# rageworx/libsrcnn

Measured on AMD Instinct MI355X. Metric: megapixels/sec SRCNN Y-channel (2x upscale), higher is better.
Workload: dtype f32

## Files before the change

### include/srcnn_amd_debug.h

```cpp
#ifndef SRCNN_AMD_DEBUG_H
#define SRCNN_AMD_DEBUG_H

#include "srcnn_amd.h"

#ifdef __cplusplus
extern "C" {
#endif
#pragma GCC visibility push(default)

#define SRCNN_MODE_RELAXED  3
#define SRCNN_RELAX_L1      1u
#define SRCNN_RELAX_L2      2u
#define SRCNN_RELAX_L3_X64  4u
#define SRCNN_RELAX_L3_F32  8u

int         srcnn_set_relaxation(unsigned mask);

int srcnn_axis_table(int filter, unsigned dst_len, unsigned src_len, int* left, int* right, double* weights);

int srcnn_fused_diag(const float* d_up, unsigned w, unsigned h, float* d_out, unsigned long long* d_dbg, void* stream);

int srcnn_debug_counts(int* tables, int* lanes);

int srcnn_debug_settings(char* buf, size_t cap, int markdown);

int srcnn_debug_clock_probe(int on);
int srcnn_debug_clock_read(int context, unsigned long long* cycles, unsigned long long* ticks, int cap);

int srcnn_debug_band_plan(unsigned r0, unsigned r1, unsigned dw, int one_of_many, unsigned* cuts, int cap);

int srcnn_debug_process_phases(double* ms, int cap);

int srcnn_debug_stream_mode(unsigned* graph_frames, unsigned* plain_frames, int* fell_back);

#pragma GCC visibility pop
#ifdef __cplusplus
}
#endif
#endif
```

### libsrcnn_amd/__init__.py

```python
import ctypes as C
import os

import numpy as np

_HERE = os.path.dirname(os.path.abspath(__file__))
LIB_PATH = os.environ.get("SRCNN_AMD_LIB") or os.path.join(_HERE, "lib", "libsrcnn_amd.so")

SRCNNF_Nearest, SRCNNF_Bilinear, SRCNNF_Bicubic, SRCNNF_Lanczos3, SRCNNF_Bspline = range(5)
MODE_STRICT, MODE_FAST, MODE_FAST_F16, MODE_RELAXED = 0, 1, 2, 3
RELAX_L1, RELAX_L2, RELAX_L3_X64, RELAX_L3_F32 = 1, 2, 4, 8

STABLE_ABI_SYMBOLS = [
    "srcnn_abi_version", "srcnn_device_count", "srcnn_init", "srcnn_init_devices", "srcnn_context_count",
    "srcnn_context_device", "srcnn_set_context", "srcnn_get_context", "srcnn_shutdown", "srcnn_trim",
    "srcnn_last_error", "srcnn_set_mode", "srcnn_get_mode", "srcnn_device_name", "srcnn_set_workspace_limit",
    "srcnn_dev_alloc", "srcnn_dev_free", "srcnn_host_alloc_pinned", "srcnn_host_free_pinned", "srcnn_memcpy_h2d",
    "srcnn_memcpy_d2h", "srcnn_memset_dev", "srcnn_stream_create", "srcnn_stream_destroy", "srcnn_stream_sync",
    "srcnn_device_sync", "srcnn_event_create", "srcnn_event_destroy", "srcnn_event_record",
    "srcnn_stream_wait_event", "srcnn_event_elapsed_ms", "srcnn_profile_enable", "srcnn_profile_reset",
    "srcnn_profile_read", "srcnn_profile_read_context", "srcnn_y_upscale2x_f32_dev",
    "srcnn_y_upscale2x_f32_batch_dev", "srcnn_y_upscale2x_f32_band_dev", "srcnn_y_upscale2x_f32_node_dev",
    "srcnn_batch_graph_create", "srcnn_batch_graph_launch", "srcnn_batch_graph_destroy", "srcnn_y_path_f32_dev",
    "srcnn_resample_f32_dev", "srcnn_conv1_f32_dev", "srcnn_conv2_f32_dev", "srcnn_conv3_f32_dev",
    "srcnn_conv12_f32_dev", "srcnn_y_upscale2x_f32", "srcnn_y_upscale2x_f32_batch", "srcnn_y_upscale2x_f32_stream",
    "srcnn_y_path_f32", "srcnn_process_u8", "srcnn_process_u8_begin", "srcnn_process_u8_wait", "srcnn_delete_array",
    "srcnn_output_size", "srcnn_comm_unique_id", "srcnn_comm_init", "srcnn_comm_destroy", "srcnn_comm_rank",
    "srcnn_comm_gather_f32", "srcnn_comm_gatherv_f32", "srcnn_comm_gatherv_at_f32",
    "srcnn_comm_tiled_y_upscale2x_f32_dev", "srcnn_band_rows", "srcnn_tiled_piece", "srcnn_comm_allgather_f32",
    "srcnn_comm_barrier", "srcnn_comm_wait", "srcnn_comm_set_timeout_ms",
]
DEBUG_SYMBOLS = [
    "srcnn_set_relaxation", "srcnn_axis_table", "srcnn_fused_diag", "srcnn_debug_counts", "srcnn_debug_settings",
    "srcnn_debug_clock_probe", "srcnn_debug_clock_read", "srcnn_debug_band_plan", "srcnn_debug_process_phases", "srcnn_debug_stream_mode",
]
YUV_SYMBOLS = ["srcnn_yuv_abi_version", "srcnn_yuv420_upscale_dev"]
YUV_EX_SYMBOLS = ["srcnn_yuv_ex_abi_version", "srcnn_yuv_plane_size", "srcnn_yuv_upscale_dev"]
RGB_SYMBOLS = ["srcnn_rgb_abi_version", "srcnn_rgb_plane_size", "srcnn_rgb_upscale_dev"]
C_ABI_SYMBOLS = STABLE_ABI_SYMBOLS + DEBUG_SYMBOLS + YUV_SYMBOLS + YUV_EX_SYMBOLS + RGB_SYMBOLS
CXX_SYMBOLS = ["_Z20ConfigureFilterSRCNN15SRCNNFilterTypeb", "_Z12ProcessSRCNNPKhjjjfRPhRjPS1_Pj"]


class YuvFormat(C.Structure):
    _fields_ = [("struct_size", C.c_uint), ("layout", C.c_int), ("chroma", C.c_int), ("depth", C.c_int), ("msb_aligned", C.c_int)]


class RgbFormat(C.Structure):
    _fields_ = [("struct_size", C.c_uint), ("layout", C.c_int), ("order", C.c_int), ("alpha", C.c_int), ("depth", C.c_int)]


class SrcnnError(RuntimeError):
    def __init__(self, code, msg):
        super().__init__("libsrcnn_amd error %d: %s" % (code, msg))
        self.code = code


_lib = None


def lib():
    global _lib
    if _lib is None:
        if not os.path.exists(LIB_PATH):
            raise ImportError("%s is missing -- run `python -m libsrcnn_amd.build` (hipcc, gfx950). "
                              "There is no CPU fallback." % LIB_PATH)
        L = C.CDLL(LIB_PATH)
        vp, u, f, sz, i = C.c_void_p, C.c_uint, C.c_float, C.c_size_t, C.c_int
        sig = {
            "srcnn_abi_version": (i, []), "srcnn_device_count": (i, []), "srcnn_init": (i, [i]),
            "srcnn_init_devices": (i, [C.POINTER(i), i]), "srcnn_context_count": (i, []), "srcnn_context_device": (i, [i]),
            "srcnn_set_context": (i, [i]), "srcnn_get_context": (i, []), "srcnn_trim": (i, []),
            "srcnn_y_upscale2x_f32_node_dev": (i, [vp, u, u, vp, i]),
            "srcnn_comm_gatherv_at_f32": (i, [vp, C.POINTER(sz), C.POINTER(sz), vp, i, vp]),
            "srcnn_comm_tiled_y_upscale2x_f32_dev": (i, [vp, u, u, vp, vp, i, i, vp]),
            "srcnn_band_rows": (i, [u, i, i, C.POINTER(u), C.POINTER(u)]),
            "srcnn_tiled_piece": (i, [u, u, i, i, i, i, C.POINTER(u), C.POINTER(u)]),
            "srcnn_debug_band_plan": (i, [u, u, u, i, C.POINTER(u), i]),
            "srcnn_shutdown": (None, []), "srcnn_last_error": (C.c_char_p, []), "srcnn_set_mode": (i, [i]),
            "srcnn_get_mode": (i, []), "srcnn_set_relaxation": (i, [u]), "srcnn_device_name": (i, [C.c_char_p, sz]),
            "srcnn_set_workspace_limit": (sz, [sz]),
            "srcnn_dev_alloc": (vp, [sz]), "srcnn_dev_free": (None, [vp]),
            "srcnn_host_alloc_pinned": (vp, [sz]), "srcnn_host_free_pinned": (None, [vp]),
            "srcnn_memcpy_h2d": (i, [vp, vp, sz, vp]), "srcnn_memcpy_d2h": (i, [vp, vp, sz, vp]),
            "srcnn_memset_dev": (i, [vp, i, sz, vp]),
            "srcnn_stream_create": (i, [C.POINTER(vp)]), "srcnn_stream_destroy": (i, [vp]),
            "srcnn_stream_sync": (i, [vp]), "srcnn_device_sync": (i, []),
            "srcnn_event_create": (i, [C.POINTER(vp)]), "srcnn_event_destroy": (i, [vp]),
            "srcnn_event_record": (i, [vp, vp]), "srcnn_event_elapsed_ms": (i, [vp, vp, C.POINTER(f)]),
            "srcnn_stream_wait_event": (i, [vp, vp]),
            "srcnn_profile_enable": (i, [i]), "srcnn_profile_reset": (i, []),
            "srcnn_profile_read": (i, [i, C.POINTER(C.c_double), C.POINTER(C.c_ulonglong)]),
            "srcnn_profile_read_context": (i, [i, i, C.POINTER(C.c_double), C.POINTER(C.c_ulonglong)]),
            "srcnn_y_upscale2x_f32_dev": (i, [vp, u, u, vp, vp]),
            "srcnn_y_upscale2x_f32_batch_dev": (i, [vp, u, u, u, vp, vp]),
            "srcnn_y_upscale2x_f32_band_dev": (i, [vp, u, u, u, u, vp, vp]),
            "srcnn_batch_graph_create": (i, [vp, u, u, u, vp, vp, C.POINTER(vp)]),
            "srcnn_batch_graph_launch": (i, [vp]), "srcnn_batch_graph_destroy": (i, [vp]),
            "srcnn_y_path_f32_dev": (i, [vp, u, u, u, u, i, vp, vp]),
            "srcnn_resample_f32_dev": (i, [vp, u, u, u, u, i, vp, vp]),
            "srcnn_conv1_f32_dev": (i, [vp, u, u, vp, vp]), "srcnn_conv2_f32_dev": (i, [vp, u, u, vp, vp]),
            "srcnn_conv3_f32_dev": (i, [vp, u, u, vp, vp]), "srcnn_conv12_f32_dev": (i, [vp, u, u, vp, vp]),
            "srcnn_y_upscale2x_f32": (i, [vp, u, u, vp]), "srcnn_y_upscale2x_f32_batch": (i, [vp, u, u, u, vp]),
            "srcnn_y_path_f32": (i, [vp, u, u, u, u, i, vp]),
            "srcnn_y_upscale2x_f32_stream": (i, [vp, u, u, u, vp, i]),
            "srcnn_process_u8": (i, [vp, u, u, u, f, i, vp, vp]),
            "srcnn_process_u8_begin": (i, [vp, u, u, u, f, i, vp, vp, C.POINTER(vp)]), "srcnn_process_u8_wait": (i, [vp]),
            "srcnn_delete_array": (None, [vp]),
            "srcnn_output_size": (i, [u, u, f, i, C.POINTER(u), C.POINTER(u)]),
            "srcnn_axis_table": (i, [i, u, u, vp, vp, vp]),
            "srcnn_comm_unique_id": (i, [vp]), "srcnn_comm_init": (i, [vp, i, i]), "srcnn_comm_destroy": (i, []),
            "srcnn_comm_gather_f32": (i, [vp, sz, vp, i, vp]), "srcnn_comm_allgather_f32": (i, [vp, sz, vp, vp]),
            "srcnn_comm_gatherv_f32": (i, [vp, C.POINTER(sz), vp, i, vp]),
            "srcnn_comm_rank": (i, [C.POINTER(i), C.POINTER(i)]),
            "srcnn_debug_counts": (i, [C.POINTER(i), C.POINTER(i)]),
            "srcnn_fused_diag": (i, [vp, u, u, vp, vp, vp]),
            "srcnn_debug_clock_probe": (i, [i]), "srcnn_debug_clock_read": (i, [i, vp, vp, i]),
            "srcnn_debug_settings": (i, [C.c_char_p, sz, i]),
            "srcnn_debug_process_phases": (i, [C.POINTER(C.c_double), i]),
            "srcnn_debug_stream_mode": (i, [C.POINTER(u), C.POINTER(u), C.POINTER(i)]),
            "srcnn_comm_barrier": (i, [vp]), "srcnn_comm_wait": (i, [vp]), "srcnn_comm_set_timeout_ms": (i, [i]),
            "srcnn_yuv_abi_version": (i, []),
            "srcnn_yuv420_upscale_dev": (i, [i, u, u, f, i, C.POINTER(vp), C.POINTER(sz), C.POINTER(vp), C.POINTER(sz), vp]),
            "srcnn_yuv_ex_abi_version": (i, []),
            "srcnn_yuv_plane_size": (i, [C.POINTER(YuvFormat), u, u, i, C.POINTER(u), C.POINTER(u), C.POINTER(sz)]),
            "srcnn_yuv_upscale_dev": (i, [C.POINTER(YuvFormat), u, u, f, i, C.POINTER(vp), C.POINTER(sz), C.POINTER(vp), C.POINTER(sz), vp]),
            "srcnn_rgb_abi_version": (i, []),
            "srcnn_rgb_plane_size": (i, [C.POINTER(RgbFormat), u, u, i, C.POINTER(u), C.POINTER(u), C.POINTER(sz)]),
            "srcnn_rgb_upscale_dev": (i, [C.POINTER(RgbFormat), u, u, f, i, C.POINTER(vp), C.POINTER(sz), C.POINTER(vp), C.POINTER(sz), vp, sz, vp]),
        }
        for name, (res, args) in sig.items():
            if name in DEBUG_SYMBOLS + YUV_SYMBOLS + YUV_EX_SYMBOLS + RGB_SYMBOLS and not hasattr(L, name) and os.environ.get("SRCNN_AMD_LIB"):
                continue
            fn = getattr(L, name)
            fn.restype, fn.argtypes = res, args
        cfg = getattr(L, CXX_SYMBOLS[0])
        cfg.restype, cfg.argtypes = None, [i, C.c_bool]
        prc = getattr(L, CXX_SYMBOLS[1])
        prc.restype = i
        prc.argtypes = [vp, u, u, u, f, C.POINTER(vp), C.POINTER(u), C.POINTER(vp), C.POINTER(u)]
        _lib = L
    return _lib


def check(rc):
    if rc != 0:
        raise SrcnnError(rc, lib().srcnn_last_error().decode("utf-8", "replace"))


def init(device=0):
    check(lib().srcnn_init(int(device)))


def init_devices(devices=None):
    if devices is None:
        check(lib().srcnn_init_devices(None, 0))
    else:
        arr = (C.c_int * len(devices))(*devices)
        check(lib().srcnn_init_devices(arr, len(devices)))
    return lib().srcnn_context_count()


def context_count():
    return lib().srcnn_context_count()


def set_context(k):
    prev = lib().srcnn_set_context(int(k))
    if prev < 0:
        raise SrcnnError(prev, lib().srcnn_last_error().decode())
    return prev


def shutdown():
    lib().srcnn_shutdown()


def device_count():
    return lib().srcnn_device_count()


def device_name():
    buf = C.create_string_buffer(256)
    check(lib().srcnn_device_name(buf, 256))
    return buf.value.decode()


def set_mode(mode):
    prev = lib().srcnn_set_mode(int(mode))
    if prev < 0:
        raise SrcnnError(prev, lib().srcnn_last_error().decode())
    return prev


def set_relaxation(mask):
    prev = lib().srcnn_set_relaxation(int(mask))
    if prev < 0:
        raise SrcnnError(prev, lib().srcnn_last_error().decode())
    return prev


def sync():
    check(lib().srcnn_device_sync())


STAGES = ("resample", "conv12", "conv3")


def profile_enable(on=True):
    return lib().srcnn_profile_enable(1 if on else 0)


def profile_reset():
    check(lib().srcnn_profile_reset())


def clock_probe(on=True):
    return lib().srcnn_debug_clock_probe(1 if on else 0)


def clock_read(context=0, cap=8192):
    cyc = np.zeros(cap, np.uint64); tk = np.zeros(cap, np.uint64)
    n = lib().srcnn_debug_clock_read(int(context), cyc.ctypes.data, tk.ctypes.data, cap)
    if n < 0:
        raise SrcnnError(n, lib().srcnn_last_error().decode())
    n = min(n, cap)
    t = np.maximum(tk[:n].astype(np.float64), 1.0)
    return [(float(c) / float(x) * 100.0, float(x) / 100.0) for c, x in zip(cyc[:n].astype(np.float64), t)]


def profile_read_context(k):
    out = {}
    for st, name in enumerate(STAGES):
        ms, n = C.c_double(), C.c_ulonglong()
        check(lib().srcnn_profile_read_context(int(k), st, C.byref(ms), C.byref(n)))
        out[name] = (ms.value, n.value)
    return out


def profile_read():
    out = {}
    for k, name in enumerate(STAGES):
        ms, n = C.c_double(0), C.c_ulonglong(0)
        check(lib().srcnn_profile_read(k, C.byref(ms), C.byref(n)))
        out[name] = (ms.value, n.value)
    return out


class DeviceBuffer:
    def __init__(self, nbytes):
        self.nbytes = int(nbytes)
        self.ptr = lib().srcnn_dev_alloc(self.nbytes)
        if not self.ptr:
            raise SrcnnError(-202, lib().srcnn_last_error().decode())

    @classmethod
    def from_numpy(cls, arr):
        arr = np.ascontiguousarray(arr)
        b = cls(arr.nbytes)
        check(lib().srcnn_memcpy_h2d(b.ptr, arr.ctypes.data, arr.nbytes, None))
        return b

    def upload(self, arr, offset=0):
        arr = np.ascontiguousarray(arr)
        assert offset + arr.nbytes <= self.nbytes
        check(lib().srcnn_memcpy_h2d(self.ptr + offset, arr.ctypes.data, arr.nbytes, None))

    def to_numpy(self, dtype, shape, offset=0):
        out = np.empty(shape, dtype)
        assert offset + out.nbytes <= self.nbytes
        check(lib().srcnn_memcpy_d2h(out.ctypes.data, self.ptr + offset, out.nbytes, None))
        return out

    def free(self):
        if self.ptr:
            lib().srcnn_dev_free(self.ptr)
            self.ptr = None

    def __del__(self):
        try:
            self.free()
        except Exception:
            pass


class Stream:
    def __init__(self):
        h = C.c_void_p()
        check(lib().srcnn_stream_create(C.byref(h)))
        self.handle = h.value

    def sync(self):
        check(lib().srcnn_stream_sync(self.handle))

    def destroy(self):
        if self.handle:
            check(lib().srcnn_stream_destroy(self.handle))
            self.handle = None


class Event:
    def __init__(self):
        h = C.c_void_p()
        check(lib().srcnn_event_create(C.byref(h)))
        self.handle = h.value

    def record(self, stream=None):
        check(lib().srcnn_event_record(self.handle, stream.handle if stream else None))

    def elapsed_ms(self, stop):
        ms = C.c_float()
        check(lib().srcnn_event_elapsed_ms(self.handle, stop.handle, C.byref(ms)))
        return ms.value


def _plane(a):
    a = np.ascontiguousarray(a, np.float32)
    assert a.ndim == 2, a.shape
    return a


def y_upscale2x(y):
    y = _plane(y)
    h, w = y.shape
    out = np.empty((2 * h, 2 * w), np.float32)
    check(lib().srcnn_y_upscale2x_f32(y.ctypes.data, w, h, out.ctypes.data))
    return out


def y_upscale2x_batch(frames):
    frames = np.ascontiguousarray(frames, np.float32)
    n, h, w = frames.shape
    out = np.empty((n, 2 * h, 2 * w), np.float32)
    check(lib().srcnn_y_upscale2x_f32_batch(frames.ctypes.data, w, h, n, out.ctypes.data))
    return out


def y_upscale2x_stream(frames, use_graph=True):
    frames = np.ascontiguousarray(frames, np.float32)
    n, h, w = frames.shape
    out = np.empty((n, 2 * h, 2 * w), np.float32)
    g = 1 if use_graph == "auto" else (int(use_graph) if isinstance(use_graph, int) and not isinstance(use_graph, bool) else (2 if use_graph else 0))
    check(lib().srcnn_y_upscale2x_f32_stream(frames.ctypes.data, w, h, n, out.ctypes.data, g))
    return out


def stream_mode():
    g, p, f = C.c_uint(0), C.c_uint(0), C.c_int(0)
    check(lib().srcnn_debug_stream_mode(C.byref(g), C.byref(p), C.byref(f)))
    return g.value, p.value, bool(f.value)


def y_path(y, dw, dh, filt=SRCNNF_Bicubic):
    y = _plane(y)
    h, w = y.shape
    out = np.empty((dh, dw), np.float32)
    check(lib().srcnn_y_path_f32(y.ctypes.data, w, h, dw, dh, filt, out.ctypes.data))
    return out


def y_upscale2x_band(y, row0, rows):
    y = _plane(y)
    h, w = y.shape
    din = DeviceBuffer.from_numpy(y)
    dout = DeviceBuffer(rows * 2 * w * 4)
    check(lib().srcnn_y_upscale2x_f32_band_dev(din.ptr, w, h, row0, rows, dout.ptr, None))
    sync()
    return dout.to_numpy(np.float32, (rows, 2 * w))


def _stage(fn, src, out_shape, *dims):
    src = np.ascontiguousarray(src, np.float32)
    din = DeviceBuffer.from_numpy(src)
    dout = DeviceBuffer(int(np.prod(out_shape)) * 4)
    check(fn(din.ptr, *dims, dout.ptr, None))
    sync()
    return dout.to_numpy(np.float32, out_shape)


def resample(y, dw, dh, filt=SRCNNF_Bicubic):
    y = _plane(y)
    h, w = y.shape
    src = DeviceBuffer.from_numpy(y)
    dst = DeviceBuffer(dw * dh * 4)
    check(lib().srcnn_resample_f32_dev(src.ptr, w, h, dw, dh, filt, dst.ptr, None))
    sync()
    return dst.to_numpy(np.float32, (dh, dw))


def conv1(y):
    y = _plane(y)
    h, w = y.shape
    return _stage(lib().srcnn_conv1_f32_dev, y, (64, h, w), w, h)


def conv2(c1):
    _, h, w = c1.shape
    return _stage(lib().srcnn_conv2_f32_dev, c1, (32, h, w), w, h)


def conv3(c2):
    _, h, w = c2.shape
    return _stage(lib().srcnn_conv3_f32_dev, c2, (h, w), w, h)


def conv12(y):
    y = _plane(y)
    h, w = y.shape
    return _stage(lib().srcnn_conv12_f32_dev, y, (32, h, w), w, h)


def axis_table(dst_len, src_len, filt=SRCNNF_Bicubic):
    win = lib().srcnn_axis_table(filt, dst_len, src_len, None, None, None)
    if win < 0:
        raise SrcnnError(win, lib().srcnn_last_error().decode())
    left = np.zeros(dst_len, np.int32)
    right = np.zeros(dst_len, np.int32)
    w = np.zeros((dst_len, win + 1), np.float64)
    lib().srcnn_axis_table(filt, dst_len, src_len, left.ctypes.data, right.ctypes.data, w.ctypes.data)
    return left, right, w


def output_size(w, h, multiply, stepscale=False):
    ow, oh = C.c_uint(0), C.c_uint(0)
    rc = lib().srcnn_output_size(w, h, float(np.float32(multiply)), 1 if stepscale else 0, C.byref(ow), C.byref(oh))
    if rc != 0:
        raise SrcnnError(rc, "srcnn_output_size")
    return ow.value, oh.value


def process_u8(rgb, multiply=2.0, filt=SRCNNF_Bicubic, want_conv=True):
    rgb = np.ascontiguousarray(rgb, np.uint8)
    h, w, d = rgb.shape
    m = np.float32(multiply)
    dw, dh = int(np.float32(w) * m), int(np.float32(h) * m)
    out = np.empty((dh, dw, d), np.uint8)
    conv = np.empty((dh, dw), np.uint8) if want_conv else None
    check(lib().srcnn_process_u8(rgb.ctypes.data, w, h, d, float(m), filt, out.ctypes.data,
                                 conv.ctypes.data if want_conv else None))
    return out, conv


YUV_I420, YUV_NV12 = 0, 1
_YUV_FORMATS = {"i420": YUV_I420, "nv12": YUV_NV12, YUV_I420: YUV_I420, YUV_NV12: YUV_NV12}


def yuv420_sizes(w, h, multiply):
    dw, dh = output_size(w, h, multiply)
    return (dw, dh), ((w + 1) // 2, (h + 1) // 2), ((dw + 1) // 2, (dh + 1) // 2)


def _addr(p):
    if p is None:
        return None
    if isinstance(p, tuple):
        base, off = p
        return _addr(base) + int(off)
    return p.ptr if isinstance(p, DeviceBuffer) else int(p)


def yuv420_upscale_dev(fmt, w, h, multiply, filt, src, src_pitch, dst, dst_pitch, stream=None):
    vp, sz = C.c_void_p, C.c_size_t
    s = (vp * 3)(*[_addr(p) for p in src])
    d = (vp * 3)(*[_addr(p) for p in dst])
    sp = (sz * 3)(*src_pitch) if src_pitch is not None else None
    dp = (sz * 3)(*dst_pitch) if dst_pitch is not None else None
    handle = stream.handle if isinstance(stream, Stream) else stream
    check(lib().srcnn_yuv420_upscale_dev(int(_YUV_FORMATS.get(fmt, fmt)), int(w), int(h), float(np.float32(multiply)), int(filt), s, sp,
                                         d, dp, handle))


def yuv420_upscale(y, u, v=None, multiply=2.0, filt=SRCNNF_Bicubic, fmt="i420", stream=None):
    fmt = _YUV_FORMATS[fmt.lower() if isinstance(fmt, str) else fmt]
    y = np.ascontiguousarray(y, np.uint8)
    h, w = y.shape
    (dw, dh), (cw, ch), (dcw, dch) = yuv420_sizes(w, h, multiply)
    if fmt == YUV_NV12:
        planes = [y, np.ascontiguousarray(u, np.uint8).reshape(ch, 2 * cw)]
        shapes = [(dh, dw), (dch, 2 * dcw)]
    else:
        planes = [y, np.ascontiguousarray(u, np.uint8), np.ascontiguousarray(v, np.uint8)]
        assert planes[1].shape == planes[2].shape == (ch, cw), (planes[1].shape, planes[2].shape, (ch, cw))
        shapes = [(dh, dw), (dch, dcw), (dch, dcw)]
    din = [DeviceBuffer.from_numpy(p) for p in planes]
    dout = [DeviceBuffer(int(np.prod(s))) for s in shapes]
    pad = [None] * (3 - len(planes))
    yuv420_upscale_dev(fmt, w, h, multiply, filt, din + pad, None, dout + pad, None, stream)
    if isinstance(stream, Stream):
        stream.sync()
    else:
        check(lib().srcnn_stream_sync(stream))
    return tuple(b.to_numpy(np.uint8, s) for b, s in zip(dout, shapes))


YUV_PLANAR, YUV_SEMIPLANAR = 0, 1
YUV_420, YUV_422, YUV_444 = 0, 1, 2
_YUV_LAYOUTS = {"planar": YUV_PLANAR, "semiplanar": YUV_SEMIPLANAR, YUV_PLANAR: YUV_PLANAR, YUV_SEMIPLANAR: YUV_SEMIPLANAR}
_YUV_CHROMAS = {"420": YUV_420, "422": YUV_422, "444": YUV_444, 420: YUV_420, 422: YUV_422, 444: YUV_444,
                YUV_420: YUV_420, YUV_422: YUV_422, YUV_444: YUV_444}


def yuv_format(layout="planar", chroma="420", depth=8, msb_aligned=False):
    layout = layout.lower() if isinstance(layout, str) else layout
    return YuvFormat(C.sizeof(YuvFormat), int(_YUV_LAYOUTS.get(layout, layout)), int(_YUV_CHROMAS.get(chroma, chroma)), int(depth),
                     int(msb_aligned))


def yuv_plane_size(fmt, w, h, plane):
    c, r, b = C.c_uint(0), C.c_uint(0), C.c_size_t(0)
    check(lib().srcnn_yuv_plane_size(C.byref(fmt), int(w), int(h), int(plane), C.byref(c), C.byref(r), C.byref(b)))
    return c.value, r.value, b.value


def yuv_plane_sizes(fmt, w, h, multiply):
    dw, dh = output_size(w, h, multiply)
    n = 2 if fmt.layout == YUV_SEMIPLANAR else 3
    return ((dw, dh), [yuv_plane_size(fmt, w, h, k) for k in range(n)], [yuv_plane_size(fmt, dw, dh, k) for k in range(n)])


def yuv_upscale_dev(fmt, w, h, multiply, filt, src, src_pitch, dst, dst_pitch, stream=None):
    vp, sz = C.c_void_p, C.c_size_t
    s = (vp * 3)(*[_addr(p) for p in src]) if src is not None else None
    d = (vp * 3)(*[_addr(p) for p in dst]) if dst is not None else None
    sp = (sz * 3)(*src_pitch) if src_pitch is not None else None
    dp = (sz * 3)(*dst_pitch) if dst_pitch is not None else None
    handle = stream.handle if isinstance(stream, Stream) else stream
    check(lib().srcnn_yuv_upscale_dev(C.byref(fmt) if fmt is not None else None, int(w), int(h), float(np.float32(multiply)),
                                      int(filt), s, sp, d, dp, handle))


def yuv_upscale(planes, layout="planar", chroma="420", depth=8, msb_aligned=False, multiply=2.0, filt=SRCNNF_Bicubic, stream=None):
    fmt = yuv_format(layout, chroma, depth, msb_aligned)
    dt = np.uint8 if depth == 8 else np.uint16
    y = np.ascontiguousarray(planes[0], dt)
    h, w = y.shape
    _, src_sizes, dst_sizes = yuv_plane_sizes(fmt, w, h, multiply)
    bps = np.dtype(dt).itemsize
    ins = [y] + [np.ascontiguousarray(p, dt).reshape(r, rb // bps) for p, (_c, r, rb) in zip(planes[1:], src_sizes[1:])]
    assert len(ins) == len(src_sizes), "%d planes given, the format has %d" % (len(ins), len(src_sizes))
    shapes = [(r, rb // bps) for (_c, r, rb) in dst_sizes]
    din = [DeviceBuffer.from_numpy(p) for p in ins]
    dout = [DeviceBuffer(max(1, int(np.prod(s)) * bps)) for s in shapes]
    pad = [None] * (3 - len(ins))
    yuv_upscale_dev(fmt, w, h, multiply, filt, din + pad, None, dout + pad, None, stream)
    if isinstance(stream, Stream):
        stream.sync()
    else:
        check(lib().srcnn_stream_sync(stream))
    return tuple(b.to_numpy(dt, s) for b, s in zip(dout, shapes))


RGB_INTERLEAVED, RGB_PLANAR = 0, 1
RGB_ORDER_RGB, RGB_ORDER_BGR = 0, 1
_RGB_LAYOUTS = {"interleaved": RGB_INTERLEAVED, "hwc": RGB_INTERLEAVED, "planar": RGB_PLANAR, "chw": RGB_PLANAR}
_RGB_ORDERS = {"rgb": RGB_ORDER_RGB, "rgba": RGB_ORDER_RGB, "bgr": RGB_ORDER_BGR, "bgra": RGB_ORDER_BGR}


def rgb_format(layout="interleaved", order="rgb", alpha=False, depth=8):
    layout = layout.lower() if isinstance(layout, str) else layout
    order = order.lower() if isinstance(order, str) else order
    return RgbFormat(C.sizeof(RgbFormat), int(_RGB_LAYOUTS.get(layout, layout)), int(_RGB_ORDERS.get(order, order)), int(alpha), int(depth))

# ... 208 lines not shown
```

### libsrcnn_amd/csrc/srcnn_capi.cpp

```cpp
#include <dlfcn.h>
#include <hip/hip_runtime.h>
#include <sys/prctl.h>
#include <sys/syscall.h>
#include <unistd.h>

#include <algorithm>
#include <cstdio>
#include <cstdlib>
#include <cstring>
#include <string>
#include <thread>

#include "resample_table.hpp"
#include <chrono>
#include <sys/auxv.h>
#include <unistd.h>

#include "srcnn_host.hpp"
#include "srcnn_yuv.h"
#include "srcnn_rgb.h"
#include "../../include/srcnn_amd_yuv.h"
#include "../../include/srcnn_amd_yuv_ex.h"
#include "../../include/srcnn_amd_rgb.h"

// ... 593 lines not shown
    if (spin_waits()) return hipEventSynchronize(e);
    const hipError_t r = poll_until_ready([&] {
        if (!query_guard) return hipEventQuery(e);
        std::lock_guard<std::mutex> lk(*query_guard);
        return hipEventQuery(e);
    });
    (void)hipGetLastError();
    return r;
}

hipError_t wait_stream(hipStream_t s)
{
    if (spin_waits()) return hipStreamSynchronize(s);
    const hipError_t r = poll_until_ready([&] { return hipStreamQuery(s); });
    (void)hipGetLastError();
    return r;
}

void parallel_memcpy(void* dst, const void* src, size_t n)
{
    const size_t kChunk = 4u << 20;
    unsigned nt = (unsigned)std::min<size_t>(8, n / kChunk);
    if (nt <= 1) { memcpy(dst, src, n); return; }
    std::vector<std::thread> th;
    const size_t per = ((n / nt) + 4095) & ~size_t(4095);
    size_t done = 0;
    try {
        for (unsigned t = 1; t < nt; ++t) {
            const size_t off = (size_t)t * per;
            if (off >= n) break;
            const size_t len = std::min(per, n - off);
            th.emplace_back([=] { memcpy((char*)dst + off, (const char*)src + off, len); });
            done = off + len;
        }
    } catch (...) {
        done = th.empty() ? 0 : done;
    }
    memcpy(dst, src, std::min(per, n));
    const size_t covered = th.empty() ? std::min(per, n) : done;
    if (covered < n) memcpy((char*)dst + covered, (const char*)src + covered, n - covered);
    for (auto& t : th) t.join();
}

void ProcLane::release_buffers()
{
    ws.release();
    if (pin_in) (void)hipHostFree(pin_in);
    if (pin_out) (void)hipHostFree(pin_out);
    pin_in = pin_out = nullptr; pin_in_n = pin_out_n = 0;
}

void ProcLane::release()
{
    release_buffers();
    for (auto e : band_events) (void)hipEventDestroy(e);
    band_events.clear();
    if (st) (void)hipStreamDestroy(st);
    if (copy_st) (void)hipStreamDestroy(copy_st);
    if (in_st) (void)hipStreamDestroy(in_st);
    st = copy_st = in_st = nullptr;
}

void NodeLane::release()
{
    ws.release();
    (void)hipFree(in); (void)hipFree(band);
    in = band = nullptr; in_n = band_n = 0;
    for (auto e : events) (void)hipEventDestroy(e);
    events.clear();
    if (st) (void)hipStreamDestroy(st);
    if (copy_st) (void)hipStreamDestroy(copy_st);
    st = copy_st = nullptr;
}

LaneLease::LaneLease(Ctx& c) : cx(&c)
{
    std::unique_lock<std::mutex> lk(c.lane_mu);
    for (;;) {
        for (auto& l : c.lanes)
            if (!l->busy) { lane = l.get(); break; }
        if (lane) break;
        if (c.lanes.size() < G.max_lanes) {
            auto l = std::make_unique<ProcLane>();
            if (hipStreamCreateWithFlags(&l->st, hipStreamNonBlocking) != hipSuccess ||
                hipStreamCreateWithFlags(&l->copy_st, hipStreamNonBlocking) != hipSuccess ||
                hipStreamCreateWithFlags(&l->in_st, hipStreamNonBlocking) != hipSuccess) {
                l->release();
                rc = fail(SRCNN_E_HIP, "could not create the streams of a ProcessSRCNN lane");
                return;
            }
            c.lanes.push_back(std::move(l));
            lane = c.lanes.back().get();
            break;
        }
        c.lane_cv.wait(lk);
    }
    lane->busy = true;
}

LaneLease::~LaneLease()
{
    if (!lane) return;
    (void)hipSetDevice(cx->device);
    (void)hipStreamSynchronize(lane->st);
    (void)hipStreamSynchronize(lane->copy_st);
    (void)hipStreamSynchronize(lane->in_st);
    { std::lock_guard<std::mutex> lk(cx->lane_mu); lane->busy = false; }
    cx->lane_cv.notify_one();
}

namespace {

struct StageTimer {
    Ctx& cx; hipStream_t s; int stage; hipEvent_t a = nullptr, b = nullptr; bool on;
    hipEvent_t take()
    {
        if (!cx.event_pool.empty()) { hipEvent_t e = cx.event_pool.back(); cx.event_pool.pop_back(); return e; }
        hipEvent_t e = nullptr;
        if (hipEventCreate(&e) != hipSuccess) return nullptr;
        return e;
    }
    StageTimer(int stage_, const Call& c) : cx(*c.cx), s(c.s), stage(stage_), on(c.timing && G.profiling.load(std::memory_order_relaxed))
    {
        if (!on) return;
        std::lock_guard<std::mutex> lk(cx.mu);
        a = take(); b = take();
        if (!a || !b) { on = false; return; }
        (void)hipEventRecord(a, s);
    }
    ~StageTimer()
    {
        if (!on) return;
        (void)hipEventRecord(b, s);
        std::lock_guard<std::mutex> lk(cx.mu);
        cx.spans.push_back(StageSpan{a, b, stage});
    }
};

void drain_spans_locked(Ctx& cx)
{
    for (auto& sp : cx.spans) {
        float ms = 0.f;
        if (hipEventSynchronize(sp.b) == hipSuccess && hipEventElapsedTime(&ms, sp.a, sp.b) == hipSuccess) {
            cx.stage_ms[sp.stage] += ms;
            cx.stage_n[sp.stage] += 1;
        }
        cx.event_pool.push_back(sp.a);
        cx.event_pool.push_back(sp.b);
    }
    cx.spans.clear();
}

void run_conv12(const Call& c, const float* Y, int W, int H, int y_row_base, int y_rows, float* C2, size_t plane, int row0,
                int rows)
{
    unsigned long long* clk = nullptr;
    if (G.clock_probe.load(std::memory_order_relaxed) && c.cx->clock_buf)
        clk = c.cx->clock_buf + 2 * (size_t)(c.cx->clock_n.fetch_add(1) % kClockSlots);
    unsigned* queue = nullptr;
    hipStreamCaptureStatus cap = hipStreamCaptureStatusNone;
    const bool foreign_capture = c.s && c.ws && !c.ws->frozen && hipStreamIsCapturing(c.s, &cap) == hipSuccess && cap == hipStreamCaptureStatusActive;
    if (foreign_capture) clk = nullptr;
    if (c.ws && settings().conv12_queue && !foreign_capture) {
        if (c.ws->queue && c.ws->queue_dirty) {
            if (hipMemsetAsync(c.ws->queue, 0, 2 * sizeof(unsigned), c.s) == hipSuccess) c.ws->queue_dirty = false;
            else (void)hipGetLastError();
        }
        if (!c.ws->queue && !c.ws->frozen) {
            void* q = nullptr;
            if (hipMalloc(&q, 2 * sizeof(unsigned)) == hipSuccess && hipMemsetAsync(q, 0, 2 * sizeof(unsigned), c.s) == hipSuccess) c.ws->queue = static_cast<unsigned*>(q);
            else { (void)hipFree(q); (void)hipGetLastError(); }
        }
        queue = c.ws->queue;
    }
    launch_conv12_mfma(Y, W, H, y_row_base, y_rows, C2, plane, row0, rows, c.relax(), c.cx->num_cus, c.s, clk, queue);
}

DevAxisTable view_of(const TableRef& t) { return t->view(); }

int resample_src_rows(Call& c, const YSource& src, unsigned sw, unsigned sh, unsigned dw, unsigned dh, int filter,
                      unsigned r0, unsigned r1, float* d_dst)
{
    Workspace& ws = *c.ws;
    hipStream_t s = c.s;
    const float* d_in = src.plane;
    if (sw == dw && sh == dh) {
        if (!d_in) return fail(SRCNN_E_UNSUPPORTED, "identity-size resample needs a float plane");
        HIP_TRY(hipMemcpyAsync(d_dst, d_in + (size_t)r0 * sw, sizeof(float) * (size_t)(r1 - r0) * sw,
                               hipMemcpyDeviceToDevice, s));
        return SRCNN_OK;
    }
    TableRef tv, th;
    int rc;
    if (dw > sw && sh != dh) {
        if ((rc = get_table(c, filter, dw, sw, th))) return rc;
        if ((rc = get_table(c, filter, dh, sh, tv))) return rc;
        if (!settings().resample_2pass &&
            launch_rs2d(src, sw, sh, d_dst, dw, dh, r0, r1 - r0, view_of(tv), view_of(th), s)) return SRCNN_OK;
    }
    if (!d_in) return fail(SRCNN_E_UNSUPPORTED, "this resample shape needs a float source plane");
    if (dw <= sw) {
        const float* mid = d_in;
        int mid_row_base = 0;
        if (sw != dw) {
            if ((rc = get_table(c, filter, dw, sw, th))) return rc;
            if (sh != dh) {
                if ((rc = get_table(c, filter, dh, sh, tv))) return rc;
                unsigned lo = 0, hi = sh;
                tv->source_span(r0, r1, lo, hi);
                hi = std::min(hi, sh);
                if (hi <= lo) return fail(SRCNN_E_UNSUPPORTED, "empty source span for rows [%u,%u)", r0, r1);
                if ((rc = grow_ws(ws, ws.tmp, ws.tmp_n, (size_t)dw * (hi - lo)))) return rc;
                launch_resample_rows(d_in + (size_t)lo * sw, sw, ws.tmp, dw, hi - lo, view_of(th), s);
                mid = ws.tmp;
                mid_row_base = (int)lo;
            } else {
                launch_resample_rows(d_in + (size_t)r0 * sw, sw, d_dst, dw, r1 - r0, view_of(th), s);
                return SRCNN_OK;
            }
        }
        if (!tv && (rc = get_table(c, filter, dh, sh, tv))) return rc;
        launch_resample_cols(mid, dw, mid_row_base, d_dst, r0, r1 - r0, view_of(tv), s);
    } else {
        if (!th && (rc = get_table(c, filter, dw, sw, th))) return rc;
        const float* mid = d_in + (size_t)r0 * sw;
        if (sh != dh) {
            if (!tv && (rc = get_table(c, filter, dh, sh, tv))) return rc;
            if ((rc = grow_ws(ws, ws.tmp, ws.tmp_n, (size_t)sw * (r1 - r0)))) return rc;
            launch_resample_cols(d_in, sw, 0, ws.tmp, r0, r1 - r0, view_of(tv), s);
            mid = ws.tmp;
        }
        launch_resample_rows(mid, sw, d_dst, dw, r1 - r0, view_of(th), s);
    }
    return SRCNN_OK;
}

}

int resample_rows_range(Call& c, const float* d_in, unsigned sw, unsigned sh, unsigned dw, unsigned dh, int filter,
                        unsigned r0, unsigned r1, float* d_dst)
{
    return resample_src_rows(c, YSource::from_plane(d_in), sw, sh, dw, dh, filter, r0, r1, d_dst);
}

int check_plane(const void* in, unsigned w, unsigned h, const void* out)
{
    if (!in || !out || w == 0 || h == 0) return fail(SRCNN_E_ARG, "NULL pointer or zero dimension");
    if ((unsigned long long)w * h > 0x7fffffffULL) return fail(SRCNN_E_UNSUPPORTED, "plane too large");
    return SRCNN_OK;
}

int y_path_rows(Call& c, const YSource& src, unsigned w, unsigned h, unsigned dw, unsigned dh, int filter,
                unsigned r0, unsigned r1, float* d_out)
{
    if (r1 > dh || r0 >= r1) return fail(SRCNN_E_ARG, "row range [%u,%u) outside 0..%u", r0, r1, dh);
    if (dh > (1u << 20) || h > (1u << 20) || dw > 0x7fffffu || (r1 - r0) > 65535u * 16u)
        return fail(SRCNN_E_UNSUPPORTED, "output %ux%u too large", dw, dh);
    Workspace& ws = *c.ws;
    [[maybe_unused]] Ctx& cx = *c.cx;
    const unsigned ca = r0 >= 2 ? r0 - 2 : 0, cb = std::min(dh, r1 + 2);
    const unsigned ua = ca >= 4 ? ca - 4 : 0, ub = std::min(dh, cb + 4);
    int rc;
    if ((rc = grow_ws(ws, ws.up, ws.up_n, (size_t)dw * (ub - ua)))) return rc;
#ifndef SRCNN_STRICT_ONLY
    const bool fused = c.mode == SRCNN_MODE_FAST_F16;
    if (fused) {
        {
            StageTimer t(SRCNN_STAGE_RESAMPLE, c);
            if ((rc = resample_src_rows(c, src, w, h, dw, dh, filter, ua, ub, ws.up))) return rc;
        }
        {
            StageTimer t(SRCNN_STAGE_CONV12, c);
            launch_fused_f16(ws.up, (int)dw, (int)dh, (int)ua, (int)(ub - ua), d_out, (int)r0, (int)(r1 - r0), cx.fused_w,
                             cx.num_cus, c.s);
        }
        HIP_TRY(hipGetLastError());
        return SRCNN_OK;
    }
#endif
    if ((rc = grow_ws(ws, ws.c2, ws.c2_n, (size_t)C2N * dw * (cb - ca)))) return rc;
    TraceRange tr("srcnn y_path rows [%u,%u) of %ux%u", r0, r1, dw, dh);
    {
        StageTimer t(SRCNN_STAGE_RESAMPLE, c);
        if ((rc = resample_src_rows(c, src, w, h, dw, dh, filter, ua, ub, ws.up))) return rc;
    }
    const size_t plane = (size_t)dw * (cb - ca);
    {
        StageTimer t(SRCNN_STAGE_CONV12, c);
        run_conv12(c, ws.up, (int)dw, (int)dh, (int)ua, (int)(ub - ua), ws.c2, plane, (int)ca, (int)(cb - ca));
    }
    {
        StageTimer t(SRCNN_STAGE_CONV3, c);
        launch_conv3(ws.c2, plane, (int)dw, (int)dh, (int)ca, (int)(cb - ca), d_out, (int)r0, (int)(r1 - r0),
                     c.relax(), c.s);
    }
    if (const hipError_t e = hipGetLastError(); e != hipSuccess) {
        ws.queue_dirty = true;
        return fail(SRCNN_E_HIP, "y_path_rows: %s", hipGetErrorString(e));
    }
    return SRCNN_OK;
}

int y_path_source_rows(Call& c, unsigned h, unsigned dh, int filter, unsigned r0, unsigned r1, unsigned& lo, unsigned& hi)
{
    const unsigned ca = r0 >= 2 ? r0 - 2 : 0, cb = std::min(dh, r1 + 2);
    const unsigned ua = ca >= 4 ? ca - 4 : 0, ub = std::min(dh, cb + 4);
    if (h == dh) { lo = ua; hi = ub; return SRCNN_OK; }
    TableRef tv;
    int rc = get_table(c, filter, dh, h, tv);
    if (rc) return rc;
    tv->source_span(ua, ub, lo, hi);
    hi = std::min(hi, h);
    return SRCNN_OK;
}

unsigned budget_band_rows(unsigned dw)
{
    const size_t budget = G.ws_budget.load();
    const size_t row_bytes = (size_t)C2N * dw * sizeof(float);
    const size_t fit = budget / row_bytes;
    return (unsigned)std::min<size_t>(std::max<size_t>(16, fit > 4 ? fit - 4 : 1), 1u << 20);
}

std::vector<unsigned> plan_cuts(unsigned R0, unsigned R1, unsigned dw, unsigned dh, const double* frac, int nfrac, int grid, int tile_rows)
{
    const unsigned rows = R1 - R0;
    std::vector<unsigned> cuts{R0};
    const unsigned tiles_x = (dw + 63) / 64;
    unsigned a = R0;
    for (int i = 0; i < nfrac; ++i) {
        const unsigned want = std::max(32u, (unsigned)(rows * frac[i]));
        unsigned b = a + (want & ~15u);
        if (grid > 0 && tile_rows > 0) {
            const unsigned top = a >= 2 ? 2 : a;
            const unsigned t_want = (want + top + 2 + tile_rows - 1) / tile_rows;
            const unsigned t_lo = std::max(1u, (unsigned)(t_want * 0.7)), t_hi = std::max(t_lo, (unsigned)(t_want * 1.3));
            double best = -1.0;
            unsigned best_t = t_want;
            for (unsigned t = t_lo; t <= t_hi; ++t) {
                const unsigned long long tiles = (unsigned long long)t * tiles_x;
                const unsigned long long rounds = (tiles + grid - 1) / grid;
                const double fill = (double)tiles / (double)(rounds * grid);
                const double score = fill - 1e-4 * (t > t_want ? t - t_want : t_want - t);
                if (score > best) { best = score; best_t = t; }
            }
            if (best_t * tile_rows > top + 2) b = a + best_t * tile_rows - top - 2;
        }
        if (b <= a || b >= R1 || R1 - b < 32) break;
        cuts.push_back(b);
        a = b;
    }
    cuts.push_back(R1);
    return cuts;
}

int y_path_range(Call& c, const float* d_in, unsigned w, unsigned h, unsigned dw, unsigned dh, int filter,
                 unsigned r0, unsigned r1, float* d_out)
{
    const size_t budget = G.ws_budget.load();
    if (r1 > dh || r0 >= r1) return fail(SRCNN_E_ARG, "row range [%u,%u) outside 0..%u", r0, r1, dh);
    const size_t row_bytes = (size_t)C2N * dw * sizeof(float);
    const bool no_planes = c.mode == SRCNN_MODE_FAST_F16;
    const YSource src = YSource::from_plane(d_in);
    if (no_planes || row_bytes * ((size_t)(r1 - r0) + 4) <= budget) return y_path_rows(c, src, w, h, dw, dh, filter, r0, r1, d_out);
    const unsigned band = budget_band_rows(dw);
    for (unsigned a = r0; a < r1; a += band) {
        const unsigned b = std::min(r1, a + band);
        int rc = y_path_rows(c, src, w, h, dw, dh, filter, a, b, d_out + (size_t)(a - r0) * dw);
        if (rc) return rc;
    }
    return SRCNN_OK;
}

int y_path_frame(Call& c, const float* d_in, unsigned w, unsigned h, unsigned dw, unsigned dh, int filter, float* d_out)
{
    return y_path_range(c, d_in, w, h, dw, dh, filter, 0, dh, d_out);
}

int check_y_path_args(const float* d_in, unsigned w, unsigned h, unsigned dw, unsigned dh, int filter, const float* d_out)
{
    int rc = check_plane(d_in, w, h, d_out);
    if (rc) return rc;
    if (dw == 0 || dh == 0) return fail(SRCNN_E_SCALE, "scaled size %ux%u", dw, dh);
    if (filter < 0 || filter > 4) return fail(SRCNN_E_ARG, "bad filter %d", filter);
    return SRCNN_OK;
}

namespace {

struct StreamCall {
    std::vector<TableRef> tables;
    Call c;
    std::unique_lock<std::mutex> lk;
    int rc = SRCNN_OK;
    explicit StreamCall(void* stream)
    {
        c.cx = ctx_for_stream(stream);
        if (!c.cx) { rc = SRCNN_E_NODEVICE; return; }
        c.s = (hipStream_t)stream;
        c.ws = workspace_for(*c.cx, c.s);
        c.mode = G.mode.load();
        c.hold = &tables;
        lk = std::unique_lock<std::mutex>(c.ws->mu);
    }
};

int batch_frames(Call& c, const float* d_in, unsigned w, unsigned h, unsigned nframes, float* d_out)
{
    const size_t in_n = (size_t)w * h, out_n = in_n * 4;
    for (unsigned f = 0; f < nframes; ++f) {
        int rc = y_path_frame(c, d_in + f * in_n, w, h, 2 * w, 2 * h, SRCNN_FILTER_BICUBIC, d_out + f * out_n);
        if (rc) return rc;
    }
    return SRCNN_OK;
}

struct BatchGraph {
    Ctx* cx = nullptr;
    hipGraphExec_t exec = nullptr;
    hipStream_t stream = nullptr;
    Workspace ws;
    std::vector<TableRef> tables;
};

void release_context(Ctx& cx)
{
    (void)hipSetDevice(cx.device);
    (void)hipDeviceSynchronize();
    {
        std::lock_guard<std::mutex> lk(cx.lane_mu);
        for (auto& l : cx.lanes) l->release();
        cx.lanes.clear();
    }
    cx.node.release();
    std::lock_guard<std::mutex> lk(cx.mu);
    cx.tables.clear();
    for (auto& kv : cx.ws) kv.second->release();
    cx.ws.clear();
    for (auto& sl : cx.slots) {
        if (sl.exec) (void)hipGraphExecDestroy(sl.exec);
        if (sl.st) (void)hipStreamDestroy(sl.st);
        if (sl.cst) (void)hipStreamDestroy(sl.cst);
        for (hipEvent_t* e : {&sl.e_in, &sl.e_k, &sl.e_out}) { if (*e) (void)hipEventDestroy(*e); *e = nullptr; }
        (void)hipFree(sl.din); (void)hipFree(sl.dout);
        sl.ws.release();
        sl.tables.clear();
        sl.graph_tables.clear();
// ... 630 lines not shown
    StreamCall sc(stream);
    if (sc.rc) return sc.rc;
    return y_path_range(sc.c, d_in, w, h, 2 * w, 2 * h, SRCNN_FILTER_BICUBIC, row0, row0 + rows, d_out_band);
}

int srcnn_profile_enable(int on) { return G.profiling.exchange(on != 0) ? 1 : 0; }

int srcnn_profile_reset(void)
{
    for (int k = 0; k < context_count(); ++k) {
        Ctx* cx = context_at(k);
        if (!cx) continue;
        (void)hipSetDevice(cx->device);
        std::lock_guard<std::mutex> lk(cx->mu);
        drain_spans_locked(*cx);
        for (int i = 0; i < SRCNN_STAGE_COUNT; ++i) { cx->stage_ms[i] = 0; cx->stage_n[i] = 0; }
    }
    if (Ctx* cx = context_at(srcnn_get_context())) (void)hipSetDevice(cx->device);
    return SRCNN_OK;
}

int srcnn_profile_read(int stage, double* total_ms, unsigned long long* launches)
{
    if (stage < 0 || stage >= SRCNN_STAGE_COUNT) return fail(SRCNN_E_ARG, "bad stage %d", stage);
    double ms = 0; unsigned long long n = 0;
    for (int k = 0; k < context_count(); ++k) {
        Ctx* cx = context_at(k);
        if (!cx) continue;
        (void)hipSetDevice(cx->device);
        std::lock_guard<std::mutex> lk(cx->mu);
        drain_spans_locked(*cx);
        ms += cx->stage_ms[stage]; n += cx->stage_n[stage];
    }
    if (Ctx* cx = context_at(srcnn_get_context())) (void)hipSetDevice(cx->device);
    if (total_ms) *total_ms = ms;
    if (launches) *launches = n;
    return SRCNN_OK;
}

int srcnn_debug_clock_probe(int on)
{
    if (int rc = ensure_init()) return rc;
    for (int k = 0; k < context_count(); ++k) {
        Ctx* cx = context_at(k);
        if (!cx) continue;
        (void)hipSetDevice(cx->device);
        if (on && !cx->clock_buf) {
            void* p = nullptr;
            if (hipMalloc(&p, sizeof(unsigned long long) * 2 * kClockSlots) != hipSuccess) return fail(SRCNN_E_DEVMEM, "clock probe buffer");
            cx->clock_buf = static_cast<unsigned long long*>(p);
        }
        if (cx->clock_buf) { (void)hipMemset(cx->clock_buf, 0, sizeof(unsigned long long) * 2 * kClockSlots); (void)hipDeviceSynchronize(); }
        cx->clock_n = 0;
    }
    if (Ctx* cur = context_at(srcnn_get_context())) (void)hipSetDevice(cur->device);
    return G.clock_probe.exchange(on != 0) ? 1 : 0;
}

int srcnn_debug_clock_read(int context, unsigned long long* cycles, unsigned long long* ticks, int cap)
{
    Ctx* cx = context_at(context);
    if (!cx || !cx->clock_buf) return fail(SRCNN_E_ARG, "no clock probe on context %d", context);
    (void)hipSetDevice(cx->device);
    HIP_TRY(hipDeviceSynchronize());
    const unsigned n = std::min(cx->clock_n.load(), kClockSlots);
    std::vector<unsigned long long> host(2 * (size_t)n);
    if (n) HIP_TRY(hipMemcpy(host.data(), cx->clock_buf, sizeof(unsigned long long) * 2 * n, hipMemcpyDeviceToHost));
    for (unsigned i = 0; i < n && (int)i < cap; ++i) {
        if (cycles) cycles[i] = host[2 * i];
        if (ticks) ticks[i] = host[2 * i + 1];
    }
    if (Ctx* cur = context_at(srcnn_get_context())) (void)hipSetDevice(cur->device);
    return (int)n;
}

int srcnn_profile_read_context(int context, int stage, double* total_ms, unsigned long long* launches)
{
    if (stage < 0 || stage >= SRCNN_STAGE_COUNT) return fail(SRCNN_E_ARG, "bad stage %d", stage);
    Ctx* cx = context_at(context);
    if (!cx) return fail(SRCNN_E_ARG, "no context %d", context);
    (void)hipSetDevice(cx->device);
    {
        std::lock_guard<std::mutex> lk(cx->mu);
        drain_spans_locked(*cx);
        if (total_ms) *total_ms = cx->stage_ms[stage];
        if (launches) *launches = cx->stage_n[stage];
    }
    if (Ctx* cur = context_at(srcnn_get_context())) (void)hipSetDevice(cur->device);
    return SRCNN_OK;
}

int srcnn_resample_f32_dev(const float* d_in, unsigned w, unsigned h, unsigned dw, unsigned dh, int filter,
                           float* d_out, void* stream)
{
    int rc;
    if ((rc = check_y_path_args(d_in, w, h, dw, dh, filter, d_out))) return rc;
    if (dh > (1u << 20) || h > (1u << 20)) return fail(SRCNN_E_UNSUPPORTED, "too many rows");
    StreamCall sc(stream);
    if (sc.rc) return sc.rc;
    rc = resample_rows_range(sc.c, d_in, w, h, dw, dh, filter, 0, dh, d_out);
    if (rc) return rc;
    HIP_TRY(hipGetLastError());
    return SRCNN_OK;
}

int srcnn_conv1_f32_dev(const float* d_y, unsigned w, unsigned h, float* d_c1, void* stream)
{
    int rc;
    if ((rc = check_plane(d_y, w, h, d_c1))) return rc;
    if (h > 65535u * 4u) return fail(SRCNN_E_UNSUPPORTED, "too many rows");
    if (!ctx_for_stream(stream)) return SRCNN_E_NODEVICE;
    launch_conv1_planes(d_y, (int)w, (int)h, d_c1, (hipStream_t)stream);
    HIP_TRY(hipGetLastError());
    return SRCNN_OK;
}

int srcnn_conv2_f32_dev(const float* d_c1, unsigned w, unsigned h, float* d_c2, void* stream)
{
    int rc;
    if ((rc = check_plane(d_c1, w, h, d_c2))) return rc;
    if (!ctx_for_stream(stream)) return SRCNN_E_NODEVICE;
    launch_conv2_planes(d_c1, (size_t)w * h, d_c2, (hipStream_t)stream);
    HIP_TRY(hipGetLastError());
    return SRCNN_OK;
}

int srcnn_conv3_f32_dev(const float* d_c2, unsigned w, unsigned h, float* d_out, void* stream)
{
    int rc;
    if ((rc = check_plane(d_c2, w, h, d_out))) return rc;
    if (h > 65535u * 16u) return fail(SRCNN_E_UNSUPPORTED, "too many rows");
    if (!ctx_for_stream(stream)) return SRCNN_E_NODEVICE;
    Call c;
    c.mode = G.mode.load();
    launch_conv3(d_c2, (size_t)w * h, (int)w, (int)h, 0, (int)h, d_out, 0, (int)h, c.relax(), (hipStream_t)stream);
    HIP_TRY(hipGetLastError());
    return SRCNN_OK;
}

int srcnn_conv12_f32_dev(const float* d_y, unsigned w, unsigned h, float* d_c2, void* stream)
{
    int rc;
    if ((rc = check_plane(d_y, w, h, d_c2))) return rc;
    if (h > 65535u * 4u) return fail(SRCNN_E_UNSUPPORTED, "too many rows");
    Call c;
    c.cx = ctx_for_stream(stream);
    if (!c.cx) return SRCNN_E_NODEVICE;
    c.s = (hipStream_t)stream; c.mode = G.mode.load();
    run_conv12(c, d_y, (int)w, (int)h, 0, (int)h, d_c2, (size_t)w * h, 0, (int)h);
    HIP_TRY(hipGetLastError());
    return SRCNN_OK;
}

int srcnn_axis_table(int filter, unsigned dst_len, unsigned src_len, int* left, int* right, double* weights)
{
    if (dst_len == 0 || src_len == 0) return fail(SRCNN_E_ARG, "zero length");
    const srcnn::AxisTable t = srcnn::build_axis_table(filter, dst_len, src_len);
    if (left) memcpy(left, t.first.data(), sizeof(int) * dst_len);
    if (right) memcpy(right, t.last.data(), sizeof(int) * dst_len);
    if (weights) memcpy(weights, t.weight.data(), sizeof(double) * t.weight.size());
    return t.window;
}

int srcnn_fused_diag(const float* d_up, unsigned w, unsigned h, float* d_out, unsigned long long* d_dbg, void* stream)
{
    int rc;
    if ((rc = check_plane(d_up, w, h, d_out))) return rc;
#ifdef SRCNN_STRICT_ONLY
    (void)d_dbg; (void)stream;
    return fail(SRCNN_E_UNSUPPORTED, "strict-only build: the fused fp16 kernel is not compiled in");
#else
    Ctx* cx = ctx_for_stream(stream);
    if (!cx) return SRCNN_E_NODEVICE;
    launch_fused_f16(d_up, (int)w, (int)h, 0, (int)h, d_out, 0, (int)h, cx->fused_w, cx->num_cus, (hipStream_t)stream, d_dbg);
    HIP_TRY(hipGetLastError());
    return SRCNN_OK;
#endif
}

int srcnn_debug_settings(char* buf, size_t cap, int markdown)
{
    const std::string t = settings().describe(markdown != 0);
    if (buf && cap) snprintf(buf, cap, "%s", t.c_str());
    return (int)t.size();
}

int srcnn_debug_counts(int* tables, int* lanes)
{
    int nt = 0, nl = 0;
    for (int k = 0; k < context_count(); ++k) {
        Ctx* cx = context_at(k);
        if (!cx) continue;
        { std::lock_guard<std::mutex> lk(cx->mu); nt += (int)cx->tables.size(); }
        { std::lock_guard<std::mutex> lk(cx->lane_mu); nl += (int)cx->lanes.size(); }
    }
    if (tables) *tables = nt;
    if (lanes) *lanes = nl;
    return SRCNN_OK;
}

int srcnn_yuv_abi_version(void) { return SRCNN_AMD_YUV_VERSION; }

int srcnn_yuv420_upscale_dev(int format, unsigned w, unsigned h, float multiply, int filter,
                             const unsigned char* const src[3], const size_t src_pitch[3],
                             unsigned char* const dst[3], const size_t dst_pitch[3], void* stream)
{
    if (format != SRCNN_YUV_I420 && format != SRCNN_YUV_NV12) return fail(SRCNN_E_ARG, "unknown YUV format %d", format);
    YuvGeom g;
    g.semi = format == SRCNN_YUV_NV12;
    unsigned dw = 0, dh = 0;
    YuvPlane in[3], out[3];
    int rc;
    if ((rc = check_yuv_args(g, w, h, multiply, filter, reinterpret_cast<const void* const*>(src), src_pitch,
                             reinterpret_cast<void* const*>(dst), dst_pitch, dw, dh, in, out))) return rc;
    StreamCall sc(stream);
    if (sc.rc) return sc.rc;
    TraceRange tr("srcnn yuv420 %ux%u -> %ux%u", w, h, dw, dh);
    return yuv_frame(sc.c, g, w, h, dw, dh, filter, in, out);
}

int srcnn_yuv_ex_abi_version(void) { return SRCNN_AMD_YUV_EX_VERSION; }

int srcnn_yuv_plane_size(const srcnn_yuv_format* fmt, unsigned w, unsigned h, int plane, unsigned* cols, unsigned* rows,
                         size_t* row_bytes)
{
    YuvGeom g;
    int rc;
    if ((rc = yuv_geom_from_format(fmt, g))) return rc;
    if (w == 0 || h == 0) return fail(SRCNN_E_ARG, "zero dimension %ux%u", w, h);
    if (plane < 0 || plane > 2) return fail(SRCNN_E_ARG, "plane %d", plane);
    unsigned pc = w, pr = h;
    size_t rb = (size_t)g.bps * w;
    if (plane > 0) {
        pc = g.ccols(w), pr = g.crows(h);
        rb = (size_t)g.bps * pc * (g.semi ? 2 : 1);
        if (g.semi && plane == 2) pc = pr = 0, rb = 0;
    }
    if (cols) *cols = pc;
    if (rows) *rows = pr;
    if (row_bytes) *row_bytes = rb;
    return SRCNN_OK;
}

int srcnn_yuv_upscale_dev(const srcnn_yuv_format* fmt, unsigned w, unsigned h, float multiply, int filter,
                          const void* const src[3], const size_t src_pitch[3],
                          void* const dst[3], const size_t dst_pitch[3], void* stream)
{
    YuvGeom g;
    unsigned dw = 0, dh = 0;
    YuvPlane in[3], out[3];
    int rc;
    if ((rc = yuv_geom_from_format(fmt, g))) return rc;
    if ((rc = check_yuv_args(g, w, h, multiply, filter, src, src_pitch, dst, dst_pitch, dw, dh, in, out))) return rc;
    StreamCall sc(stream);
    if (sc.rc) return sc.rc;
    TraceRange tr("srcnn yuv %ux%u -> %ux%u", w, h, dw, dh);
    return yuv_frame(sc.c, g, w, h, dw, dh, filter, in, out);
}

int srcnn_rgb_abi_version(void) { return SRCNN_AMD_RGB_VERSION; }

int srcnn_rgb_plane_size(const srcnn_rgb_format* fmt, unsigned w, unsigned h, int plane, unsigned* cols, unsigned* rows,
                         size_t* row_bytes)
{
    RgbRule g;
    int rc;
    if ((rc = rgb_rule_from_format(fmt, g))) return rc;
    if (w == 0 || h == 0) return fail(SRCNN_E_ARG, "zero dimension %ux%u", w, h);
    if (plane < 0 || plane > 3) return fail(SRCNN_E_ARG, "plane %d", plane);
    const bool used = g.planar ? plane < g.ch : plane == 0;
    if (cols) *cols = used ? w : 0;
    if (rows) *rows = used ? h : 0;
    if (row_bytes) *row_bytes = used ? (size_t)g.bps * w * (g.planar ? 1 : g.ch) : 0;
    return SRCNN_OK;
}

int srcnn_rgb_upscale_dev(const srcnn_rgb_format* fmt, unsigned w, unsigned h, float multiply, int filter,
                          const void* const src[4], const size_t src_pitch[4], void* const dst[4], const size_t dst_pitch[4],
                          void* dst_conv, size_t dst_conv_pitch, void* stream)
{
    RgbRule g;
    unsigned dw = 0, dh = 0;
    YuvPlane in[4], out[5], conv;
    int rc;
    if ((rc = rgb_rule_from_format(fmt, g))) return rc;
    if ((rc = check_rgb_args(g, w, h, multiply, filter, src, src_pitch, dst, dst_pitch, dst_conv, dst_conv_pitch, dw, dh, in, out, conv))) return rc;
    StreamCall sc(stream);
    if (sc.rc) return sc.rc;
    TraceRange tr("srcnn rgb %ux%u -> %ux%u", w, h, dw, dh);
    return rgb_frame(sc.c, g, w, h, dw, dh, filter, in, out, conv);
}

}
```

### libsrcnn_amd/csrc/srcnn_kernels.h

```cpp
#pragma once
#include <hip/hip_runtime.h>
#include <stddef.h>

namespace srcnn {

constexpr int C1N = 64;
constexpr int C2N = 32;
enum : int {
    RELAX_L1 = 1,
    RELAX_L2 = 2,
    RELAX_L3_X64 = 4,
    RELAX_L3_F32 = 8,
    RELAX_FAST = RELAX_L1 | RELAX_L2 | RELAX_L3_F32
};
constexpr int kWeightCount = 64 + 64 * 81 + 32 + 32 * 64 + 1 + 32 * 25;

struct DevWeights {
    float w1t[81][C1N];
    float b1[C1N];
    float w2[C2N][C1N];
    float b2[C2N];
    float w3[C2N][25];
    float b3;
    float pad_[3];
    float w3p[C2N * 30];
};

struct DevAxisTable {
    const int* first;
    const int* taps;
    const double* weight;
    int stride;
    int max_taps;
    int monotone;
    const int* h_first;
    const int* h_taps;
};

struct YSource {
    const float* plane = nullptr;
    const unsigned char* rgb = nullptr;
    int depth = 0;
    static YSource from_plane(const float* p) { YSource y; y.plane = p; return y; }
    static YSource from_rgb(const unsigned char* p, int d) { YSource y; y.rgb = p; y.depth = d; return y; }
};

#ifndef FU_NW_DEF
#define FU_NW_DEF 8
#endif
constexpr int FU_NK = 5;
constexpr int FU_NW = FU_NW_DEF;
struct FusedF16Weights {
    unsigned short w1[FU_NK][2][2][64][8];
    unsigned short w2[2][2][2][64][8];
    unsigned short w3[2][2][64][8];
    float b1[64];
    float b2[32];
    float w88[64];
    float b3;
    float pad_[3];
};

hipError_t upload_weights(const DevWeights& w);
hipError_t fused_f16_prepare();
void launch_fused_f16(const float* Y, int W, int H, int y_row_base, int y_rows, float* out, int out_row0, int out_rows,
                      const FusedF16Weights* d_blob, int num_cus, hipStream_t s, unsigned long long* dbg = nullptr);

void launch_resample_cols(const float* src, int w, int src_row_base, float* dst, int dst_row0, int dst_rows,
                          const DevAxisTable& t, hipStream_t s);
void launch_resample_rows(const float* src, int src_w, float* dst, int dst_w, int rows, const DevAxisTable& t,
                          hipStream_t s);
bool launch_rs2d(const YSource& src, int src_w, int src_h, float* dst, int dst_w, int dst_h, int dst_row0, int dst_rows,
                 const DevAxisTable& tv, const DevAxisTable& th, hipStream_t s);
hipError_t rs2d_prepare();
bool rs2d_fits(int np, int src_w, int src_h, int dst_w, int dst_h, int r0, int r1, const DevAxisTable& tv, const DevAxisTable& th);
bool launch_merge_fused(const unsigned char* rgb_src, int src_w, int src_h, int depth, const float* Yp,
                        unsigned char* rgb_out, unsigned char* conv_opt, int dst_w, int dst_h, int dst_row0, int dst_rows,
                        const DevAxisTable& tv, const DevAxisTable& th, hipStream_t s);
hipError_t conv12_mfma_prepare();
void launch_conv12_mfma(const float* Y, int W, int H, int y_row_base, int y_rows, float* C2, size_t plane_stride, int out_row0,
                        int out_rows, int relax, int num_cus, hipStream_t s, unsigned long long* clk = nullptr,
                        unsigned* queue = nullptr);
void conv12_grid_info(int num_cus, int* blocks, int* tile_rows);
constexpr int kConv12TileRows = 16, kConv12BlocksPerCU = 2;
void launch_conv3(const float* C2, size_t plane_stride, int W, int H, int c2_row_base, int c2_rows, float* out,
                  int out_row0, int out_rows, int relax, hipStream_t s);
void launch_conv1_planes(const float* Y, int W, int H, float* C1, hipStream_t s);
void launch_conv2_planes(const float* C1, size_t n, float* C2v, hipStream_t s);
void launch_rgb_split(const unsigned char* rgb, size_t n, int d, float* Yp, float* Cb, float* Cr, float* A,
                      hipStream_t s);
void launch_ycc_merge(const float* Yp, const float* Cb, const float* Cr, const float* A, size_t n, int d,
                      unsigned char* rgb, unsigned char* conv_opt, hipStream_t s);

}
```

### libsrcnn_amd/csrc/srcnn_kernels.hip

```cpp
#include <hip/hip_runtime.h>
#include <type_traits>
#include <stdint.h>
#include <stdlib.h>
#include <algorithm>
#include "srcnn_kernels.h"
#include "srcnn_settings.hpp"

#pragma clang fp contract(off)

namespace srcnn {

__constant__ DevWeights cW;

hipError_t upload_weights(const DevWeights& w)
{
    return hipMemcpyToSymbol(HIP_SYMBOL(cW), &w, sizeof(DevWeights));
}

__device__ __forceinline__ int clampi(int v, int lo, int hi) { return v < lo ? lo : (v > hi ? hi : v); }

__global__ __launch_bounds__(256) void k_resample_cols(
    const float* __restrict__ src, int w, int src_row_base,
    float* __restrict__ dst, int dst_row0, int dst_rows,
    const int* __restrict__ first, const int* __restrict__ taps, const double* __restrict__ wt, int stride)
// ... 316 lines not shown
    const int xl = min(x0t + 256, a.dst_w) - 1;
    const int c0 = rs_sload(a.hfirst, x0t), cn = rs_sload(a.hfirst, xl) + rs_sload(a.htaps, xl) - c0;
    const int chunks = (cn + 63) >> 6;

    const int wr_r = tid / MAXT, wr_t = tid - wr_r * MAXT;
    double wreg = 0.0;
    int freg = 0, nreg = 0;
    auto fetch = [&](int sub) {
        const int ry0 = (blockIdx.y * a.tpb + sub) * TH;
        const int rows = min(TH, a.dst_rows - ry0);
        const int y0 = a.dst_row0 + ry0, yl = y0 + rows - 1;
        const int vmin = rs_sload(a.vfirst, y0), nsrc = rs_sload(a.vfirst, yl) + rs_sload(a.vtaps, yl) - vmin;
        if (tid < TH * MAXT && wr_r < rows) {
            const int y = y0 + wr_r;
            nreg = a.vtaps[y];
            freg = a.vfirst[y] - vmin;
            wreg = a.vwt[(size_t)y * a.vstride + min(wr_t, a.vstride - 1)];
        }
        float* raw = raw2 + (sub & 1) * raw_plane;
        const float* g = a.src_plane + (size_t)vmin * a.src_w + c0 + lane;
        for (int r = wv; r < nsrc; r += 4)
            for (int ch = 0; ch < chunks; ++ch)
                if (ch * 64 + lane < cn) rs_dma_dword(g + (size_t)r * a.src_w + ch * 64, raw + r * LW + ch * 64);
    };

    fetch(0);


    const double* hp[4][MAXT];
    double w[4][MAXT];
    int nmax = 0;
#pragma unroll
    for (int j = 0; j < 4; ++j) {
        const int xc = min(x0t + 128 * (j >> 1) + 2 * lane + (j & 1), a.dst_w - 1);
        const int s0 = a.hfirst[xc] - c0, n = a.htaps[xc];
        const double* wr = a.hwt + (size_t)xc * a.hstride;
        nmax = max(nmax, n);
#pragma unroll
        for (int t = 0; t < MAXT; ++t) {
            w[j][t] = t < n ? wr[t] : 0.0;
            hp[j][t] = mid + wv * LW + (t < n ? s0 + t : ZC);
        }
    }
    if (tid < TH) mid[tid * LW + ZC] = 0.0;
    const bool short_taps = MAXT > 1 && __builtin_amdgcn_ballot_w64(nmax > MAXT - 1) == 0;

    const int xa = x0t + 2 * lane, xb = xa + 128;
    for (int sub = 0; sub < a.tpb; ++sub) {
        const int ry0 = (blockIdx.y * a.tpb + sub) * TH;
        if (ry0 >= a.dst_rows) break;
        const int rows = min(TH, a.dst_rows - ry0);
        double* vw = vw2 + (sub & 1) * TH * MAXT;
        int* vf = vf2 + (sub & 1) * TH;
        int* vn = vn2 + (sub & 1) * TH;
        const float* raw = raw2 + (sub & 1) * raw_plane;
        if (tid < TH * MAXT && wr_r < rows) {
            vw[tid] = wr_t < nreg ? wreg : 0.0;
            if (wr_t == 0) { vf[wr_r] = freg; vn[wr_r] = nreg; }
        }
        asm volatile("s_waitcnt vmcnt(0)" ::: "memory");
        __syncthreads();
        if (sub + 1 < a.tpb && ry0 + TH < a.dst_rows) fetch(sub + 1);

        const int full = cn & ~63, rem = cn - full;
        const bool tail = rem > 0 && rem <= 16;
        const int cv = tail ? full : cn;
        for (int r = wv; r < rows; r += 4) {
            const int rb = __builtin_amdgcn_readfirstlane(vf[r]), cnt = __builtin_amdgcn_readfirstlane(vn[r]);
            double* mrow = mid + r * LW;
            const double* vwr = vw + r * MAXT;
            switch (cnt) {
#define RS_V(N) case N: if constexpr (N <= MAXT) rs_vertical_row<N, 1, MAXT, LW, double>(raw, raw_plane, mrow, vwr, rb, cv, lane); break;
            RS_V(1) RS_V(2) RS_V(3) RS_V(4) RS_V(5) RS_V(6) RS_V(7) RS_V(8)
#undef RS_V
            default: break;
            }
        }
        if (tail) {
            const int r = wv + 4 * (lane >> 4), c = full + (lane & 15);
            if (r < rows && c < cn) {
                const int rb = vf[r], cnt = vn[r];
                const double* vwr = vw + r * MAXT;
                double acc = 0.0;
#pragma unroll
                for (int t = 0; t < MAXT; ++t) {
                    const bool on = t < cnt;
                    const float xv = raw[(rb + (on ? t : 0)) * LW + c];
                    acc = acc + vwr[t] * (double)(on ? xv : 0.f);
                }
                mid[r * LW + c] = (double)(float)acc;
            }
        }
        __builtin_amdgcn_fence(__ATOMIC_RELEASE, "wavefront");
        __builtin_amdgcn_wave_barrier();
        __builtin_amdgcn_fence(__ATOMIC_ACQUIRE, "wavefront");
        auto horizontal = [&](auto ntaps) {
            constexpr int NT = decltype(ntaps)::value;
#pragma unroll
            for (int k = 0; k < RPT; ++k) {
                const int r = wv + 4 * k;
                if (r >= rows) break;
                float o[4];
#pragma unroll
                for (int j = 0; j < 4; ++j) {
                    double xs[NT];
#pragma unroll
                    for (int t = 0; t < NT; ++t) xs[t] = hp[j][t][4 * k * LW];
                    double acc = 0.0;
#pragma unroll
                    for (int t = 0; t < NT; ++t) acc = acc + w[j][t] * xs[t];
                    o[j] = (float)acc;
                }
                float* dr = a.dst + (size_t)(ry0 + r) * a.dst_w;
                if (a.vec) {
                    *reinterpret_cast<float2*>(dr + xa) = make_float2(o[0], o[1]);
                    if (xb < a.dst_w) *reinterpret_cast<float2*>(dr + xb) = make_float2(o[2], o[3]);
                } else {
                    if (xa < a.dst_w) dr[xa] = o[0];
                    if (xa + 1 < a.dst_w) dr[xa + 1] = o[1];
                    if (xb < a.dst_w) dr[xb] = o[2];
                    if (xb + 1 < a.dst_w) dr[xb + 1] = o[3];
                }
            }
        };
        if (xa < a.dst_w) {
            if (short_taps) horizontal(std::integral_constant<int, (MAXT > 1 ? MAXT - 1 : 1)>{});
            else horizontal(std::integral_constant<int, MAXT>{});
        }
        __builtin_amdgcn_fence(__ATOMIC_RELEASE, "wavefront");
        __builtin_amdgcn_wave_barrier();
        __builtin_amdgcn_fence(__ATOMIC_ACQUIRE, "wavefront");
    }
}

#define PIN(v) asm volatile("" : "+v"(v))
typedef float f32x32 __attribute__((ext_vector_type(32)));
typedef float f32x16 __attribute__((ext_vector_type(16)));

constexpr int M_NW = 8;
constexpr int M_TW = 64, M_TH = 2 * M_NW;
constexpr int M_LW = M_TW + 8;
constexpr int M_W1 = 81 * 64, M_W2 = 32 * 64, M_B1 = 64, M_B2 = 32;
constexpr int M_C1 = 32 * 32;
constexpr int M_YT = (M_TH + 8) * M_LW;
constexpr int M_BPC = 2;
static_assert(M_TH == kConv12TileRows && M_BPC == kConv12BlocksPerCU, "srcnn_kernels.h carries this geometry for the band planners");
constexpr int m_ybufs(bool ld) { return ld ? 2 : 1; }
constexpr int m_lds_floats(bool ld) { return M_W1 + M_W2 + M_B1 + M_B2 + m_ybufs(ld) * M_YT + M_NW * M_C1 + 2; }

template <int RELAX, bool LD>
__global__ __launch_bounds__(64 * M_NW, 4) void k_conv12_mfma(
    const float* __restrict__ Y, int W, int H, int y_row_base, int y_rows,
    float* __restrict__ C2, size_t plane_stride, int out_row0, int out_rows, int tiles_x, int ntiles,
    unsigned long long* __restrict__ clk, unsigned* __restrict__ queue)
{
    constexpr int NW = M_NW, NT = 64 * NW, TH = M_TH, YT = M_YT;
    unsigned long long clk_c0 = 0, clk_r0 = 0;
    if (clk && blockIdx.x == 0) { clk_c0 = __builtin_amdgcn_s_memtime(); clk_r0 = __builtin_amdgcn_s_memrealtime(); }
    constexpr bool STRICT1 = !(RELAX & 1), STRICT2 = !(RELAX & 2);
    extern __shared__ __attribute__((aligned(16))) float lds[];
    float* W1s = lds;
    float* W2s = W1s + M_W1;
    float* B1s = W2s + M_W2;
    float* B2s = B1s + M_B1;
    float* Yt  = B2s + M_B2;
    float* C1s = Yt + m_ybufs(LD) * YT;

    const int tid = threadIdx.x, lane = tid & 63, wv = tid >> 6, half = lane >> 5, col = lane & 31;

    constexpr bool WDMA = LD;
    const int wave_e0w = __builtin_amdgcn_readfirstlane(tid & ~63);
    if constexpr (WDMA) {
#pragma unroll
        for (int i = 0; i < (M_W1 + NT - 1) / NT; ++i) {
            const int e = tid + i * NT;
            if (e < M_W1) rs_dma_dword(&cW.w1t[0][0] + e, W1s + i * NT + wave_e0w);
        }
#pragma unroll
        for (int i = 0; i < (M_W2 + NT - 1) / NT; ++i) {
            const int e = tid + i * NT;
            if (e < M_W2) { const int fp = e >> 6, l = e & 63; rs_dma_dword(&cW.w2[l & 31][2 * fp + (l >> 5)], W2s + i * NT + wave_e0w); }
        }
        if (tid < 64) {
            const int hf = tid >> 5, r = tid & 31;
            rs_dma_dword(&cW.b1[32 * (r >> 4) + 8 * ((r & 15) >> 2) + 4 * hf + (r & 3)], B1s);
        }
        if (tid < 32) {
            const int hf = tid >> 4, r = tid & 15;
            rs_dma_dword(&cW.b2[8 * (r >> 2) + 4 * hf + (r & 3)], B2s);
        }
    } else {
        for (int e = tid; e < M_W1; e += NT) W1s[e] = (&cW.w1t[0][0])[e];
        for (int e = tid; e < M_W2; e += NT) {
            const int fp = e >> 6, l = e & 63;
            W2s[e] = cW.w2[l & 31][2 * fp + (l >> 5)];
        }
        if (tid < 64) {
            const int hf = tid >> 5, r = tid & 31;
            B1s[tid] = cW.b1[32 * (r >> 4) + 8 * ((r & 15) >> 2) + 4 * hf + (r & 3)];
        }
        if (tid < 32) {
            const int hf = tid >> 4, r = tid & 15;
            B2s[tid] = cW.b2[8 * (r >> 2) + 4 * hf + (r & 3)];
        }
    }
    float* myC1 = C1s + wv * M_C1;
    const f32x32 zero32 = {};

    const int full = (ntiles / (int)gridDim.x) * (int)gridDim.x;
    const int nitems = full + 4 * (ntiles - full);
    constexpr bool DMA = LD;
    constexpr int NPRE = (YT + NT - 1) / NT;
    auto tile_of = [&](int item, int& s0, int& s1) {
        int tile = item; s0 = 0; s1 = 4;
        if (item >= full) { const int i = item - full; tile = full + (i >> 2); s0 = i & 3; s1 = s0 + 1; }
        return tile;
    };
    const int wave_e0 = wave_e0w;
    auto request = [&](int item, float* buf) {
        int q0, q1;
        const int tile = tile_of(item, q0, q1);
        const int tyi = tile / tiles_x, txi = tile - tyi * tiles_x;
        const int tx0 = txi * M_TW, ty0 = out_row0 + tyi * TH;
#pragma unroll
        for (int i = 0; i < NPRE; ++i) {
            const int e = tid + i * NT;
            if (e < YT) {
                const int r = e / M_LW, c = e - r * M_LW;
                const int gy = clampi(clampi(ty0 + r - 4, 0, H - 1), y_row_base, y_row_base + y_rows - 1), gx = clampi(tx0 + c - 4, 0, W - 1);
                rs_dma_dword(Y + (size_t)(gy - y_row_base) * W + gx, buf + i * NT + wave_e0);
            }
        }
    };
    int* qslot = reinterpret_cast<int*>(C1s + NW * M_C1);
    const bool dyn = DMA && queue != nullptr;
    int it = 0;
    int item = blockIdx.x;
    if constexpr (DMA) {
        if (item < nitems) request(item, Yt);
        if (dyn && tid == 0 && item < nitems) qslot[0] = (int)gridDim.x + (int)atomicAdd(queue, 1u);
    }
    for (; item < nitems; ++it) {
        int s0, s1;
        const int tile = tile_of(item, s0, s1);
        const int tyi = tile / tiles_x, txi = tile - tyi * tiles_x;
        const int tx0 = txi * M_TW, ty0 = out_row0 + tyi * TH;
        const float* Ytc = Yt;
        int next_item = item + (int)gridDim.x;
        int drawn = 0x7fffffff;
        if constexpr (DMA) {
            Ytc = Yt + (it & 1) * YT;
            asm volatile("s_waitcnt vmcnt(0)" ::: "memory");
            __syncthreads();
            if (dyn) next_item = __builtin_amdgcn_readfirstlane(qslot[it & 1]);
            if (next_item < nitems) request(next_item, Yt + ((it + 1) & 1) * YT);
            if (dyn && tid == 0 && next_item < nitems) drawn = (int)gridDim.x + (int)atomicAdd(queue, 1u);
        } else {
            __syncthreads();
            for (int e = tid; e < YT; e += NT) {
                const int r = e / M_LW, c = e - r * M_LW;
                const int gy = clampi(clampi(ty0 + r - 4, 0, H - 1), y_row_base, y_row_base + y_rows - 1), gx = clampi(tx0 + c - 4, 0, W - 1);
                Yt[e] = Y[(size_t)(gy - y_row_base) * W + gx];
            }
            __syncthreads();
        }

#pragma unroll 1
        for (int s = s0; s < s1; ++s) {
            const int sg = wv * 4 + s;
            const int trow = sg >> 1, seg = sg & 1;
            const float* yrow = Ytc + trow * M_LW + seg * 32 + col;

            f32x32 acc = zero32;
            if constexpr (!STRICT1) {
#pragma unroll
                for (int t = 0; t < 81; ++t) {
                    const float a = W1s[t * 64 + lane];
                    const float b = yrow[(t / 9) * M_LW + (t % 9)];
                    acc = __builtin_amdgcn_mfma_f32_32x32x1f32(a, b, acc, 0, 0, 0);
                }
            } else {
                float a1 = W1s[lane], b1 = yrow[0];
                float a2 = W1s[64 + lane], b2 = yrow[1];
#pragma unroll
                for (int t = 0; t < 81; ++t) {
                    f32x32 d = __builtin_amdgcn_mfma_f32_32x32x1f32(a1, b1, zero32, 0, 0, 0);
                    PIN(d);
                    a1 = a2; b1 = b2;
                    if (t + 2 < 81) {
                        a2 = W1s[(t + 2) * 64 + lane];
                        b2 = yrow[((t + 2) / 9) * M_LW + ((t + 2) % 9)];
                    }
                    if (t == 0) acc = d; else acc += d;
                    PIN(acc);
                    __builtin_amdgcn_sched_barrier(0);
                }
            }
            f32x16 acc2 = {};
#pragma unroll
            for (int blk = 0; blk < 2; ++blk) {
#pragma unroll
                for (int r = 0; r < 16; ++r) {
                    const float v = fmaxf(acc[16 * blk + r] + B1s[half * 32 + 16 * blk + r], 0.f);
                    const int f = 8 * (r >> 2) + (r & 3);
                    myC1[(f + 4 * half) * 32 + col] = v;
                }
                __builtin_amdgcn_fence(__ATOMIC_RELEASE, "wavefront");
                __builtin_amdgcn_wave_barrier();
                __builtin_amdgcn_fence(__ATOMIC_ACQUIRE, "wavefront");

                const float* w2p = W2s + blk * 16 * 64;
                float a1 = w2p[lane], b1 = myC1[lane];
                float a2 = w2p[64 + lane], b2 = myC1[64 + lane];
                if constexpr (!STRICT2) {
#pragma unroll
                    for (int fp = 0; fp < 16; ++fp)
                        acc2 = __builtin_amdgcn_mfma_f32_32x32x2f32(w2p[fp * 64 + lane], myC1[fp * 64 + lane], acc2, 0, 0, 0);
                } else {
#pragma unroll
                    for (int fp = 0; fp < 16; ++fp) {
                        f32x32 d = __builtin_amdgcn_mfma_f32_32x32x1f32(a1, b1, zero32, 0, 0, 0);
                        PIN(d);
                        a1 = a2; b1 = b2;
                        if (fp + 2 < 16) { a2 = w2p[(fp + 2) * 64 + lane]; b2 = myC1[(fp + 2) * 64 + lane]; }
                        if (blk == 0 && fp == 0) acc2 = __builtin_shufflevector(d, d, 0, 1, 2, 3, 4, 5, 6, 7, 8, 9, 10, 11, 12, 13, 14, 15);
                        else
                        acc2 += __builtin_shufflevector(d, d, 0, 1, 2, 3, 4, 5, 6, 7, 8, 9, 10, 11, 12, 13, 14, 15);
                        acc2 += __builtin_shufflevector(d, d, 16, 17, 18, 19, 20, 21, 22, 23, 24, 25, 26, 27, 28, 29, 30, 31);
                        PIN(acc2);
                        __builtin_amdgcn_sched_barrier(0);
                    }
                }
                __builtin_amdgcn_wave_barrier();
            }

            const int row = ty0 + trow, x = tx0 + seg * 32 + col;
            if (row < out_row0 + out_rows && row < H && x < W) {
                float* dst = C2 + (size_t)(row - out_row0) * W + x;
#pragma unroll
                for (int r = 0; r < 16; ++r) {
                    const int m = 8 * (r >> 2) + (r & 3);
                    dst[(size_t)(m + 4 * half) * plane_stride] = fmaxf(acc2[r] + B2s[half * 16 + r], 0.f);
                }
            }
        }
        if (dyn && tid == 0) qslot[(it + 1) & 1] = drawn;
        item = next_item;
    }
    if (dyn && tid == 0) {
        if (atomicAdd(queue + 1, 1u) == gridDim.x - 1) { queue[0] = 0u; queue[1] = 0u; }
    }
    if (clk && blockIdx.x == 0) {
        __syncthreads();
        if (threadIdx.x == 0) {
            clk[0] = __builtin_amdgcn_s_memtime() - clk_c0;
            clk[1] = __builtin_amdgcn_s_memrealtime() - clk_r0;
        }
    }
}

constexpr int C3_TW = 64, C3_TH = 16;
constexpr int C3_LW = C3_TW + 4, C3_LH = C3_TH + 4;
constexpr int C3_CH = C3_LH * C3_LW;
static_assert(C3_LH % 4 == 0, "row slots");
constexpr int c3_mc(bool sdma) { return sdma ? 2 : 4; }

template <bool STRICT, bool OFF64 = false, bool X64 = false, bool SDMA = false>
__global__ __launch_bounds__(256, SDMA ? 6 : 3) void k_conv3(
    const float* __restrict__ C2, size_t plane_stride, int W, int H, int c2_row_base, int c2_rows,
    float* __restrict__ out, int out_row0, int out_rows, int weights_by_dma)
{
    constexpr int C3_MC = c3_mc(SDMA);
    constexpr int C3_BODY = C3_MC * C3_LH / 4;
    constexpr int C3_HALO = (C3_MC * C3_LH * 4 + 255) / 256;
    __shared__ float tile[2][C3_MC * C3_CH];
    __shared__ __attribute__((aligned(16))) float w3s[X64 ? C2N * 50 : C2N * 30];

    const int tx0 = blockIdx.x * C3_TW;
    const int ty0 = out_row0 + blockIdx.y * C3_TH;
    const int tid = threadIdx.x, lane = tid & 63, wv = tid >> 6;
    const int c2_last = c2_row_base + c2_rows - 1;
    if constexpr (X64) {
        double* w3d = reinterpret_cast<double*>(w3s);
        for (int e = tid; e < C2N * 25; e += 256) w3d[e] = (double)(&cW.w3[0][0])[e];
    } else if constexpr (STRICT) {
        const int wave_e0 = __builtin_amdgcn_readfirstlane(tid & ~63);
        if (SDMA || weights_by_dma) {
#pragma unroll
            for (int i = 0; i < (C2N * 30 + 255) / 256; ++i) {
                const int e = tid + i * 256;
                if (e < C2N * 30) rs_dma_dword(cW.w3p + e, w3s + i * 256 + wave_e0);
            }
        } else {
            for (int e = tid; e < C2N * 30; e += 256) w3s[e] = cW.w3p[e];
        }
    }

    const int bx = min(tx0 + lane, W - 1);
    const int hrow = tid >> 2, hq = tid & 3;
    const int hx = clampi(tx0 + (hq < 2 ? hq - 2 : 62 + hq), 0, W - 1);
    const int hlc = hq < 2 ? hq : 64 + hq;

    float body[C3_BODY], halo[C3_HALO];

    auto row_of = [&](int r) {
        int gy = clampi(ty0 + r - 2, 0, H - 1);
        gy = clampi(gy, c2_row_base, c2_last);
        return gy - c2_row_base;
    };
    using offs_t = std::conditional_t<OFF64, size_t, unsigned>;
    offs_t boff[C3_LH / 4], hoff[C3_HALO];
    int hm[C3_HALO];
#pragma unroll
    for (int j = 0; j < C3_LH / 4; ++j) boff[j] = ((offs_t)row_of(4 * j + wv) * (offs_t)W + (offs_t)bx) * 4u;
#pragma unroll
    for (int i = 0; i < C3_HALO; ++i) {
        const int rr = min(hrow + 64 * i, C3_MC * C3_LH - 1);
        hm[i] = rr / C3_LH;
        hoff[i] = ((offs_t)row_of(rr - hm[i] * C3_LH) * (offs_t)W + (offs_t)hx) * 4u;
    }
    const int wv_s = __builtin_amdgcn_readfirstlane(wv);
    float halo4[C3_MC];
    const int h4row = min(tid >> 2, C3_LH - 1);
    const unsigned h4off = ((unsigned)row_of(h4row) * (unsigned)W + (unsigned)hx) * 4u;
    auto issue_dma = [&](int mc, float* dst) {
        if (tid < C3_LH * 4) {
#pragma unroll
            for (int m = 0; m < C3_MC; ++m)
                halo4[m] = *reinterpret_cast<const float*>(reinterpret_cast<const char*>(C2 + (size_t)(mc + m) * plane_stride) + h4off);
        }
#pragma unroll
        for (int m = 0; m < C3_MC; ++m) {
            const unsigned long long pb = reinterpret_cast<unsigned long long>(C2 + (size_t)(mc + m) * plane_stride);
            const unsigned ub_hi = (unsigned)__builtin_amdgcn_readfirstlane((int)(unsigned)(pb >> 32));
            const unsigned ub_lo = (unsigned)__builtin_amdgcn_readfirstlane((int)(unsigned)pb);
            const unsigned long long ub = ((unsigned long long)ub_hi << 32) | (unsigned long long)ub_lo;
#pragma unroll
            for (int j = 0; j < C3_LH / 4; ++j) {
                const int i = m * (C3_LH / 4) + j;
                if constexpr (!OFF64)
                    rs_dma_dword_s(reinterpret_cast<const void*>(ub), boff[j], dst + (wv_s + 4 * i) * C3_LW + 2);
            }
        }
    };
    auto land_dma = [&](float* dst) {
        if (tid < C3_LH * 4) {
#pragma unroll
            for (int m = 0; m < C3_MC; ++m) dst[m * C3_CH + h4row * C3_LW + hlc] = halo4[m];
        }
        asm volatile("s_waitcnt vmcnt(0)" ::: "memory");
    };
    auto issue = [&](int mc) {
#pragma unroll
        for (int i = 0; i < C3_BODY; ++i) {
            const int m = i / (C3_LH / 4), j = i % (C3_LH / 4);
            const char* plane = reinterpret_cast<const char*>(C2 + (size_t)(mc + m) * plane_stride);
            body[i] = *reinterpret_cast<const float*>(plane + boff[j]);
        }
#pragma unroll
        for (int i = 0; i < C3_HALO; ++i) {
            const int rr = hrow + 64 * i;
            if (rr < C3_MC * C3_LH)
                halo[i] = *reinterpret_cast<const float*>(reinterpret_cast<const char*>(C2 + ((size_t)mc + hm[i]) * plane_stride) + hoff[i]);
        }
    };
    auto land = [&](float* dst) {
#pragma unroll
        for (int i = 0; i < C3_BODY; ++i) dst[(wv + 4 * i) * C3_LW + 2 + lane] = body[i];
#pragma unroll
        for (int i = 0; i < C3_HALO; ++i) {
            const int rr = hrow + 64 * i;
            if (rr < C3_MC * C3_LH) dst[rr * C3_LW + hlc] = halo[i];
        }
    };

    float sum[4] = {0.f, 0.f, 0.f, 0.f};

    if constexpr (SDMA) { issue_dma(0, tile[0]); land_dma(tile[0]); }
    else { issue(0); land(tile[0]); }
    if constexpr (STRICT) asm volatile("s_waitcnt vmcnt(0)" ::: "memory");
    __syncthreads();

    const int offA = (wv * 4) * C3_LW + lane;
    int offB = offA + 4 * C3_LW;
    asm volatile("" : "+v"(offB));

#pragma unroll 1
    for (int c = 0; c < C2N / C3_MC; ++c) {
        const float* cur = tile[c & 1];
        if (c + 1 < C2N / C3_MC) {
            if constexpr (SDMA) issue_dma((c + 1) * C3_MC, tile[(c + 1) & 1]);
            else issue((c + 1) * C3_MC);
        }
#pragma unroll 1
        for (int m = 0; m < C3_MC; ++m) {
            const float* t = cur + m * C3_CH + (wv * 4) * C3_LW + lane;
            if constexpr (X64) {
                const double* wd = reinterpret_cast<const double*>(w3s) + (c * C3_MC + m) * 25;
                double a[4] = {0.0, 0.0, 0.0, 0.0};
#pragma unroll
                for (int r = 0; r < 8; ++r) {
                    double v[5];
#pragma unroll
                    for (int cc = 0; cc < 5; ++cc) v[cc] = (double)t[r * C3_LW + cc];
#pragma unroll
                    for (int q = 0; q < 4; ++q) {
                        const int dy = r - q;
                        if (dy >= 0 && dy < 5) {
#pragma unroll
                            for (int dx = 0; dx < 5; ++dx) a[q] = __builtin_fma(wd[dy * 5 + dx], v[dx], a[q]);
                        }
                    }
                }
#pragma unroll
                for (int q = 0; q < 4; ++q) sum[q] = (float)((double)sum[q] + a[q]);
            } else if constexpr (STRICT && SDMA) {
                typedef float f2 __attribute__((ext_vector_type(2)));
                const float* tA = cur + m * C3_CH + offA;
                const float* tB = cur + m * C3_CH + offB;
                f2 va[8], vb[8], vp[7];
#pragma unroll
                for (int r = 0; r < 4; ++r) {
                    va[r] = f2{tA[r * C3_LW + 0], tA[r * C3_LW + 1]};
                    vb[r] = f2{tA[r * C3_LW + 2], tA[r * C3_LW + 3]};
                    va[r + 4] = f2{tB[r * C3_LW + 0], tB[r * C3_LW + 1]};
                    vb[r + 4] = f2{tB[r * C3_LW + 2], tB[r * C3_LW + 3]};
                }
#pragma unroll
                for (int k = 0; k < 3; ++k) {
                    vp[k] = f2{tA[k * C3_LW + 4], tA[(k + 1) * C3_LW + 4]};
                    vp[k + 4] = f2{tB[k * C3_LW + 4], tB[(k + 1) * C3_LW + 4]};
                }
                vp[3] = f2{tA[3 * C3_LW + 4], tB[4]};
                const float* wrow = w3s + (c * C3_MC + m) * 30;
                double a[4] = {0.0, 0.0, 0.0, 0.0};
#pragma unroll
                for (int dy = 0; dy < 5; ++dy) {
                    const f2 wa = f2{wrow[dy * 6 + 0], wrow[dy * 6 + 1]};
                    const f2 wb = f2{wrow[dy * 6 + 2], wrow[dy * 6 + 3]};
                    const f2 wc = f2{wrow[dy * 6 + 4], wrow[dy * 6 + 4]};
                    const f2 pc01 = wc * vp[dy], pc23 = wc * vp[dy + 2];
#pragma unroll
                    for (int q = 0; q < 4; ++q) {
                        const f2 pa = wa * va[q + dy], pb = wb * vb[q + dy];
                        const float pc = q == 0 ? pc01.x : q == 1 ? pc01.y : q == 2 ? pc23.x : pc23.y;
                        a[q] = (dy == 0) ? (double)pa.x : a[q] + (double)pa.x;
                        a[q] = a[q] + (double)pa.y;
                        a[q] = a[q] + (double)pb.x;
                        a[q] = a[q] + (double)pb.y;
                        a[q] = a[q] + (double)pc;
                    }
                }
#pragma unroll
                for (int q = 0; q < 4; ++q) sum[q] = (float)((double)sum[q] + a[q]);
            } else if constexpr (STRICT) {
                typedef float f2 __attribute__((ext_vector_type(2)));
                f2 va[8], vb[8];
                float vc[8];
#pragma unroll
                for (int r = 0; r < 8; ++r) {
                    va[r] = f2{t[r * C3_LW + 0], t[r * C3_LW + 1]};
                    vb[r] = f2{t[r * C3_LW + 2], t[r * C3_LW + 3]};
                    vc[r] = t[r * C3_LW + 4];
                }
                const float* wrow = w3s + (c * C3_MC + m) * 30;
                double a[4] = {0.0, 0.0, 0.0, 0.0};
#pragma unroll
                for (int dy = 0; dy < 5; ++dy) {
                    const f2 wa = f2{wrow[dy * 6 + 0], wrow[dy * 6 + 1]};
                    const f2 wb = f2{wrow[dy * 6 + 2], wrow[dy * 6 + 3]};
                    const float wc = wrow[dy * 6 + 4];
#pragma unroll
                    for (int q = 0; q < 4; ++q) {
                        const f2 pa = wa * va[q + dy], pb = wb * vb[q + dy];
                        const float pc = wc * vc[q + dy];
                        a[q] = (dy == 0) ? (double)pa.x : a[q] + (double)pa.x;
                        a[q] = a[q] + (double)pa.y;
                        a[q] = a[q] + (double)pb.x;
                        a[q] = a[q] + (double)pb.y;
                        a[q] = a[q] + (double)pc;
                    }
                }
#pragma unroll
                for (int q = 0; q < 4; ++q) sum[q] = (float)((double)sum[q] + a[q]);
            } else {
                const float* wm = cW.w3[c * C3_MC + m];
                float win[8][5];
#pragma unroll
                for (int r = 0; r < 8; ++r)
#pragma unroll
                    for (int cc = 0; cc < 5; ++cc) win[r][cc] = t[r * C3_LW + cc];
#pragma unroll
                for (int q = 0; q < 4; ++q) {
                    float a = 0.f;
#pragma unroll
                    for (int dy = 0; dy < 5; ++dy)
#pragma unroll
                        for (int dx = 0; dx < 5; ++dx) a = __builtin_fmaf(wm[dy * 5 + dx], win[q + dy][dx], a);
                    sum[q] += a;
                }
            }
        }
        if (c + 1 < C2N / C3_MC) {
            if constexpr (SDMA) land_dma(tile[(c + 1) & 1]);
            else land(tile[(c + 1) & 1]);
        }
        __syncthreads();
    }
    const int x = tx0 + lane;
#pragma unroll
    for (int q = 0; q < 4; ++q) {
        const int row = ty0 + wv * 4 + q;
        if (x < W && row < H && row < out_row0 + out_rows) {
            float v = sum[q] + cW.b3;
            v = fminf(fmaxf(v, 0.f), 255.f);
            out[(size_t)(row - out_row0) * W + x] = v;
        }
    }
}

#ifndef SRCNN_STRICT_ONLY
constexpr int CF_TW = 128, CF_TH = 16, CF_MC = 2;
constexpr int CF_LW = CF_TW + 4, CF_LH = CF_TH + 4;
constexpr int CF_CH = CF_LH * CF_LW;
constexpr int CF_BODY = CF_MC * CF_LH / 2;

__global__ __launch_bounds__(256) void k_conv3_fast(
    const float* __restrict__ C2, size_t plane_stride, int W, int H, int c2_row_base, int c2_rows,
    float* __restrict__ out, int out_row0, int out_rows)
{
    __shared__ __attribute__((aligned(16))) float tile[2][CF_MC * CF_CH];

    const int tx0 = blockIdx.x * CF_TW;
    const int ty0 = out_row0 + blockIdx.y * CF_TH;
    const int tid = threadIdx.x, lane = tid & 63, wv = tid >> 6;
    const int c2_last = c2_row_base + c2_rows - 1;

    const int bcol = tid & 127, bslot = tid >> 7;
    const int bx = min(tx0 + bcol, W - 1);
    const int hrow = tid >> 2, hq = tid & 3;
    const int hx = clampi(tx0 + (hq < 2 ? hq - 2 : 126 + hq), 0, W - 1);
    const int hlc = hq < 2 ? hq : 128 + hq;

    float body[CF_BODY], halo = 0.f;
    auto row_of = [&](int r) {
        int gy = clampi(ty0 + r - 2, 0, H - 1);
        gy = clampi(gy, c2_row_base, c2_last);
        return gy - c2_row_base;
    };
    auto issue = [&](int mc) {
#pragma unroll
        for (int i = 0; i < CF_BODY; ++i) {
            const int m = i / (CF_LH / 2), r = 2 * (i % (CF_LH / 2)) + bslot;
            body[i] = C2[(size_t)(mc + m) * plane_stride + (size_t)row_of(r) * W + bx];
        }
        if (hrow < CF_MC * CF_LH) {
            const int m = hrow / CF_LH, r = hrow - m * CF_LH;
            halo = C2[(size_t)(mc + m) * plane_stride + (size_t)row_of(r) * W + hx];
        }
    };
    auto land = [&](float* dst) {
#pragma unroll
        for (int i = 0; i < CF_BODY; ++i) dst[(2 * i + bslot) * CF_LW + 2 + bcol] = body[i];
        if (hrow < CF_MC * CF_LH) dst[hrow * CF_LW + hlc] = halo;
    };

    float sum[4][2] = {};
    issue(0);
    land(tile[0]);
    __syncthreads();
#pragma unroll 1
    for (int c = 0; c < C2N / CF_MC; ++c) {
        const float* cur = tile[c & 1];
        if (c + 1 < C2N / CF_MC) issue((c + 1) * CF_MC);
#pragma unroll 1
        for (int m = 0; m < CF_MC; ++m) {
            const float* t = cur + m * CF_CH + (wv * 4) * CF_LW + 2 * lane;
            const float* wm = cW.w3[c * CF_MC + m];
            float win[8][6];
#pragma unroll
            for (int r = 0; r < 8; ++r)
#pragma unroll
                for (int p = 0; p < 3; ++p) {
                    const float2 v = *reinterpret_cast<const float2*>(t + r * CF_LW + 2 * p);
                    win[r][2 * p] = v.x; win[r][2 * p + 1] = v.y;
                }
            float a[4][2] = {};
#pragma unroll
            for (int dy = 0; dy < 5; ++dy)
#pragma unroll
                for (int dx = 0; dx < 5; ++dx) {
                    const float wgt = wm[dy * 5 + dx];
#pragma unroll
                    for (int q = 0; q < 4; ++q) {
                        a[q][0] = __builtin_fmaf(wgt, win[q + dy][dx], a[q][0]);
                        a[q][1] = __builtin_fmaf(wgt, win[q + dy][dx + 1], a[q][1]);
                    }
                }
#pragma unroll
            for (int q = 0; q < 4; ++q) { sum[q][0] += a[q][0]; sum[q][1] += a[q][1]; }
        }
        if (c + 1 < C2N / CF_MC) land(tile[(c + 1) & 1]);
        __syncthreads();
    }
#pragma unroll
    for (int q = 0; q < 4; ++q) {
        const int row = ty0 + wv * 4 + q;
        if (row < H && row < out_row0 + out_rows) {
#pragma unroll
            for (int e = 0; e < 2; ++e) {
                const int x = tx0 + 2 * lane + e;
                if (x < W) out[(size_t)(row - out_row0) * W + x] = fminf(fmaxf(sum[q][e] + cW.b3, 0.f), 255.f);
            }
        }
    }
}

#endif

__global__ __launch_bounds__(256) void k_conv1_planes(const float* __restrict__ Y, int W, int H,
                                                      float* __restrict__ C1, size_t plane_stride)
{
    const int x = blockIdx.x * 64 + (threadIdx.x & 63);
    const int y = blockIdx.y * 4 + (threadIdx.x >> 6);
    const int k0 = blockIdx.z * 8;
    if (x >= W || y >= H) return;
    float acc[8] = {0, 0, 0, 0, 0, 0, 0, 0};
    for (int i = 0; i < 9; ++i) {
        const int gy = clampi(y + i - 4, 0, H - 1);
        for (int j = 0; j < 9; ++j) {
            const float v = Y[(size_t)gy * W + clampi(x + j - 4, 0, W - 1)];
#pragma unroll
            for (int k = 0; k < 8; ++k) acc[k] = acc[k] + cW.w1t[i * 9 + j][k0 + k] * v;
        }
    }
#pragma unroll
    for (int k = 0; k < 8; ++k)
        C1[(size_t)(k0 + k) * plane_stride + (size_t)y * W + x] = fmaxf(acc[k] + cW.b1[k0 + k], 0.f);
}

__global__ __launch_bounds__(256) void k_conv2_planes(const float* __restrict__ C1, size_t n,
                                                      float* __restrict__ C2v)
{
    const size_t p = (size_t)blockIdx.x * 256 + threadIdx.x;
    const int m0 = blockIdx.y * 8;
    if (p >= n) return;
    float acc[8] = {0, 0, 0, 0, 0, 0, 0, 0};
    for (int f = 0; f < C1N; ++f) {
        const float v = C1[(size_t)f * n + p];
#pragma unroll
        for (int m = 0; m < 8; ++m) acc[m] = acc[m] + v * cW.w2[m0 + m][f];
    }
#pragma unroll
    for (int m = 0; m < 8; ++m) C2v[(size_t)(m0 + m) * n + p] = fmaxf(acc[m] + cW.b2[m0 + m], 0.f);
}

__global__ __launch_bounds__(256) void k_rgb_split(const unsigned char* __restrict__ rgb, size_t n, int d,
                                                   float* __restrict__ Yp, float* __restrict__ Cb,
                                                   float* __restrict__ Cr, float* __restrict__ A)
{
// ... 44 lines not shown
static inline bool aligned_to(const void* p, unsigned a) { return (reinterpret_cast<uintptr_t>(p) & (a - 1)) == 0; }

namespace {
constexpr int RS_LDS_LIMIT = 96 * 1024;

struct Rs2dPlan { int lw = 0, sr = 0, maxt = 0, tpb = 1; size_t lds = 0; unsigned gx = 0, gy = 0; bool ok = false; };

Rs2dPlan rs2d_plan(int np, int dst_w, int dst_row0, int dst_rows, const DevAxisTable& tv, const DevAxisTable& th, bool sliding = false)
{
    Rs2dPlan p;
    if (dst_rows <= 0 || dst_w <= 0 || !tv.monotone || !th.monotone || !tv.h_first || !th.h_first) return p;
    const int m = std::max(tv.max_taps, th.max_taps);
    if (m > 8) return p;
    p.maxt = m <= 3 ? 3 : (m <= 5 ? 5 : 8);
    int span = 0;
    for (int x0 = 0; x0 < dst_w; x0 += 256) {
        const int xl = std::min(x0 + 256, dst_w) - 1;
        span = std::max(span, th.h_first[xl] + th.h_taps[xl] - th.h_first[x0]);
    }
    p.lw = span + 1 <= 136 ? 136 : (span + 1 <= 272 ? 272 : 0);
    for (int r = 0; r < dst_rows; r += (sliding ? 1 : RS_TH)) {
        const int y0 = dst_row0 + r, yl = dst_row0 + std::min(r + RS_TH, dst_rows) - 1;
        p.sr = std::max(p.sr, tv.h_first[yl] + tv.h_taps[yl] - tv.h_first[y0]);
    }
    p.lds = (size_t)rs_lds_bytes(np, p.maxt, p.sr, p.lw);
    const unsigned tiles_y = cdiv(dst_rows, RS_TH);
    p.gx = cdiv(dst_w, 256);
    const int tpb_env = (int)settings().rs_tpb;
    p.tpb = tpb_env > 0 ? std::min(tpb_env, RS_MAX_TPB) : (int)std::max(1u, std::min<unsigned>(RS_MAX_TPB, cdiv(p.gx * tiles_y, 1024u)));
    p.gy = cdiv(tiles_y, p.tpb);
    p.ok = p.lw > 0 && p.sr > 0 && p.lds <= (size_t)RS_LDS_LIMIT && p.gy <= 65535u;
    return p;
}

template <int KIND, int D, bool CONV, class F>
void rs2d_variants(F&& f)
{
#define RS_ONE(MT, LW_) f(reinterpret_cast<const void*>(&k_rs2d<KIND, D, MT, LW_, CONV>), MT, LW_);
    RS_ONE(3, 136) RS_ONE(5, 136) RS_ONE(8, 136) RS_ONE(3, 272) RS_ONE(5, 272) RS_ONE(8, 272)
#undef RS_ONE
}

template <int KIND, int D, bool CONV>
void rs2d_dispatch(const Rs2dPlan& p, const Rs2dArgs& a, hipStream_t s)
{
    const dim3 grid(p.gx, p.gy), block(256);
#define RS_GO(MT, LW_) hipLaunchKernelGGL((k_rs2d<KIND, D, MT, LW_, CONV>), grid, block, p.lds, s, a)
    if (p.lw == 136) { if (p.maxt == 3) RS_GO(3, 136); else if (p.maxt == 5) RS_GO(5, 136); else RS_GO(8, 136); }
    else             { if (p.maxt == 3) RS_GO(3, 272); else if (p.maxt == 5) RS_GO(5, 272); else RS_GO(8, 272); }
#undef RS_GO
}
}

hipError_t rs2d_prepare()
{
    hipError_t err = hipSuccess;
    auto raise = [&](const void* fn, int, int) {
        const hipError_t e = hipFuncSetAttribute(fn, hipFuncAttributeMaxDynamicSharedMemorySize, RS_LDS_LIMIT);
        if (e != hipSuccess && err == hipSuccess) err = e;
    };
    rs2d_variants<0, 3, false>(raise);
#define RS_ONE(MT, LW_) raise(reinterpret_cast<const void*>(&k_rs2d_dma<MT, LW_>), MT, LW_);
    RS_ONE(3, 136) RS_ONE(5, 136) RS_ONE(8, 136) RS_ONE(3, 272) RS_ONE(5, 272) RS_ONE(8, 272)
#undef RS_ONE
    rs2d_variants<1, 3, false>(raise); rs2d_variants<1, 4, false>(raise);
    rs2d_variants<2, 3, false>(raise); rs2d_variants<2, 3, true>(raise);
    rs2d_variants<2, 4, false>(raise); rs2d_variants<2, 4, true>(raise);
    return err;
}

bool rs2d_fits(int np, int src_w, int src_h, int dst_w, int dst_h, int r0, int r1, const DevAxisTable& tv, const DevAxisTable& th)
{
    if (dst_w < src_w || dst_h < src_h || r1 <= r0) return false;
    const Rs2dPlan p = rs2d_plan(np, dst_w, r0, r1 - r0, tv, th, true);
    return p.lw > 0 && p.sr > 0 && p.maxt > 0 && p.lds <= (size_t)RS_LDS_LIMIT;
}

bool launch_rs2d(const YSource& src, int src_w, int src_h, float* dst, int dst_w, int dst_h, int dst_row0, int dst_rows,
                 const DevAxisTable& tv, const DevAxisTable& th, hipStream_t s)
{
    if (dst_w < src_w || dst_h < src_h) return false;
    if (!src.plane && !(src.rgb && (src.depth == 3 || src.depth == 4))) return false;
    const Rs2dPlan p = rs2d_plan(1, dst_w, dst_row0, dst_rows, tv, th);
    if (!p.ok) return false;
    Rs2dArgs a{};
    a.src_plane = src.plane; a.src_rgb = src.rgb; a.src_w = src_w;
    a.dst = dst; a.dst_w = dst_w; a.dst_row0 = dst_row0; a.dst_rows = dst_rows;
    a.sr = p.sr; a.tpb = p.tpb;
    a.vfirst = tv.first; a.vtaps = tv.taps; a.vwt = tv.weight; a.vstride = tv.stride;
    a.hfirst = th.first; a.htaps = th.taps; a.hwt = th.weight; a.hstride = th.stride;
    a.vec = (dst_w % 4 == 0) && aligned_to(dst, 16);
    const bool dma = settings().rs_dma;
    const size_t lds_dma = p.lds + (size_t)RS_TH * p.lw * 4;
    if (src.plane && dma && lds_dma <= (size_t)64 * 1024) {
        const dim3 grid(p.gx, p.gy), block(256);
#define RS_GO(MT, LW_) hipLaunchKernelGGL((k_rs2d_dma<MT, LW_>), grid, block, lds_dma, s, a)
        if (p.lw == 136) { if (p.maxt == 3) RS_GO(3, 136); else if (p.maxt == 5) RS_GO(5, 136); else RS_GO(8, 136); }
        else             { if (p.maxt == 3) RS_GO(3, 272); else if (p.maxt == 5) RS_GO(5, 272); else RS_GO(8, 272); }
#undef RS_GO
    }
    else if (src.plane) rs2d_dispatch<0, 3, false>(p, a, s);
    else if (src.depth == 3) rs2d_dispatch<1, 3, false>(p, a, s);
    else rs2d_dispatch<1, 4, false>(p, a, s);
    return true;
}

bool launch_merge_fused(const unsigned char* rgb_src, int src_w, int src_h, int depth, const float* Yp,
                        unsigned char* rgb_out, unsigned char* conv_opt, int dst_w, int dst_h, int dst_row0, int dst_rows,
                        const DevAxisTable& tv, const DevAxisTable& th, hipStream_t s)
{
    if (dst_w < src_w || dst_h < src_h || (depth != 3 && depth != 4)) return false;
    const Rs2dPlan p = rs2d_plan(depth - 1, dst_w, dst_row0, dst_rows, tv, th);
    if (!p.ok) return false;
    Rs2dArgs a{};
    a.src_rgb = rgb_src; a.src_w = src_w;
    a.yp = Yp; a.out_rgb = rgb_out; a.out_conv = conv_opt;
    a.dst_w = dst_w; a.dst_row0 = dst_row0; a.dst_rows = dst_rows;
    a.sr = p.sr; a.tpb = p.tpb;
    a.vfirst = tv.first; a.vtaps = tv.taps; a.vwt = tv.weight; a.vstride = tv.stride;
    a.hfirst = th.first; a.htaps = th.taps; a.hwt = th.weight; a.hstride = th.stride;
    a.vec = (dst_w % 4 == 0) && aligned_to(Yp, 16) && aligned_to(rgb_out, 4) && (!conv_opt || aligned_to(conv_opt, 4));
    if (depth == 3) { if (conv_opt) rs2d_dispatch<2, 3, true>(p, a, s); else rs2d_dispatch<2, 3, false>(p, a, s); }
    else            { if (conv_opt) rs2d_dispatch<2, 4, true>(p, a, s); else rs2d_dispatch<2, 4, false>(p, a, s); }
    return true;
}

template <int RELAX, bool LD>
static hipError_t prep_one()
{
    return hipFuncSetAttribute(reinterpret_cast<const void*>(&k_conv12_mfma<RELAX, LD>),
                               hipFuncAttributeMaxDynamicSharedMemorySize, (int)(sizeof(float) * m_lds_floats(LD)));
}

hipError_t conv12_mfma_prepare()
{
    hipError_t e;
    if ((e = prep_one<0, true>()) != hipSuccess) return e;
    if ((e = prep_one<0, false>()) != hipSuccess) return e;
#ifndef SRCNN_STRICT_ONLY
    if ((e = prep_one<1, true>()) != hipSuccess) return e;
    if ((e = prep_one<2, true>()) != hipSuccess) return e;
    if ((e = prep_one<3, true>()) != hipSuccess) return e;
#endif
    return hipSuccess;
}

void conv12_grid_info(int num_cus, int* blocks, int* tile_rows)
{
    if (blocks) *blocks = M_BPC * num_cus;
    if (tile_rows) *tile_rows = M_TH;
}

void launch_conv12_mfma(const float* Y, int W, int H, int y_row_base, int y_rows, float* C2, size_t plane_stride, int out_row0,
                        int out_rows, int relax, int num_cus, hipStream_t s, unsigned long long* clk, unsigned* queue)
{
    if (out_rows <= 0) return;
    const int tiles_x = (int)cdiv(W, M_TW), tiles_y = (int)cdiv(out_rows, M_TH);
    const int ntiles = tiles_x * tiles_y;
    const int cap = M_BPC * num_cus;
    const int grid = ntiles >= cap ? cap : (settings().conv12_spread ? std::min(4 * ntiles, cap) : ntiles);
#define CONV12_GO(R, LD) hipLaunchKernelGGL((k_conv12_mfma<R, LD>), dim3(grid), dim3(64 * M_NW), sizeof(float) * m_lds_floats(LD), s, Y, W, H, \
                                           y_row_base, y_rows, C2, plane_stride, out_row0, out_rows, tiles_x, ntiles, clk, LD ? queue : nullptr)
#ifdef SRCNN_STRICT_ONLY
    (void)relax;
    if (settings().conv12_dma) CONV12_GO(0, true); else CONV12_GO(0, false);
#else
    switch (relax & 3) {
    case 0: if (settings().conv12_dma) CONV12_GO(0, true); else CONV12_GO(0, false); break;
    case 1: CONV12_GO(1, true); break;
    case 2: CONV12_GO(2, true); break;
    default: CONV12_GO(3, true); break;
    }
#endif
#undef CONV12_GO
}

void launch_conv3(const float* C2, size_t plane_stride, int W, int H, int c2_row_base, int c2_rows, float* out,
                  int out_row0, int out_rows, int relax, hipStream_t s)
{
    if (out_rows <= 0) return;
#ifndef SRCNN_STRICT_ONLY
    const bool strict = !(relax & (RELAX_L3_X64 | RELAX_L3_F32));
    const bool wide_planes = (size_t)c2_rows * (size_t)W * sizeof(float) >= ((size_t)1 << 32);
    if (relax & RELAX_L3_X64) {
        const dim3 gx(cdiv(W, 64), cdiv(out_rows, 16));
        if (wide_planes)
            hipLaunchKernelGGL((k_conv3<true, true, true>), gx, dim3(256), 0, s, C2, plane_stride, W, H, c2_row_base, c2_rows, out, out_row0, out_rows, 0);
        else
            hipLaunchKernelGGL((k_conv3<true, false, true>), gx, dim3(256), 0, s, C2, plane_stride, W, H, c2_row_base, c2_rows, out, out_row0, out_rows, 0);
        return;
    }
    if (!strict) {
        dim3 gridf(cdiv(W, CF_TW), cdiv(out_rows, CF_TH));
        hipLaunchKernelGGL(k_conv3_fast, gridf, dim3(256), 0, s, C2, plane_stride, W, H, c2_row_base, c2_rows, out,
                           out_row0, out_rows);
        return;
    }
#else
    (void)relax;
#endif
    dim3 grid(cdiv(W, 64), cdiv(out_rows, 16));
    const bool force_wide = settings().conv3_off64;
    const int wdma = settings().conv3_wdma ? 1 : 0;
    const bool wide = force_wide || (size_t)c2_rows * (size_t)W * sizeof(float) >= ((size_t)1 << 32);
    if (!wide && wdma)
        hipLaunchKernelGGL((k_conv3<true, false, false, true>), grid, dim3(256), 0, s, C2, plane_stride, W, H, c2_row_base, c2_rows,
                           out, out_row0, out_rows, 1);
    else if (!wide)
        hipLaunchKernelGGL((k_conv3<true, false>), grid, dim3(256), 0, s, C2, plane_stride, W, H, c2_row_base, c2_rows,
                           out, out_row0, out_rows, wdma);
    else
        hipLaunchKernelGGL((k_conv3<true, true>), grid, dim3(256), 0, s, C2, plane_stride, W, H, c2_row_base, c2_rows,
                           out, out_row0, out_rows, wdma);
}

void launch_conv1_planes(const float* Y, int W, int H, float* C1, hipStream_t s)
{
    dim3 grid(cdiv(W, 64), cdiv(H, 4), C1N / 8);
    hipLaunchKernelGGL(k_conv1_planes, grid, dim3(256), 0, s, Y, W, H, C1, (size_t)W * H);
}

void launch_conv2_planes(const float* C1, size_t n, float* C2v, hipStream_t s)
{
    dim3 grid((unsigned)((n + 255) / 256), C2N / 8);
    hipLaunchKernelGGL(k_conv2_planes, grid, dim3(256), 0, s, C1, n, C2v);
}

template <int D>
__global__ __launch_bounds__(256) void k_rgb_split4(const unsigned* __restrict__ rgb32, size_t n4,
                                                    float4* __restrict__ Yp, float4* __restrict__ Cb,
                                                    float4* __restrict__ Cr, float4* __restrict__ A)
{
    const size_t q = (size_t)blockIdx.x * 256 + threadIdx.x;
    if (q >= n4) return;
    unsigned wds[D];
#pragma unroll
    for (int k = 0; k < D; ++k) wds[k] = rgb32[q * D + k];
    float yv[4], cbv[4], crv[4], av[4];
#pragma unroll
    for (int i = 0; i < 4; ++i) {
        float ch[4] = {0.f, 0.f, 0.f, 0.f};
#pragma unroll
        for (int k = 0; k < D; ++k) {
            const int byte = i * D + k;
            ch[k] = (float)((wds[byte >> 2] >> (8 * (byte & 3))) & 0xffu);
        }
        const float r = ch[0], g = ch[1], b = ch[2];
        yv[i] = (0.299f * r) + (0.587f * g) + (0.114f * b);
        cbv[i] = 128.f - (0.1687f * r) - (0.3313f * g) + (0.5f * b);
        crv[i] = 128.f + (0.5f * r) - (0.4187f * g) - (0.0813f * b);
        av[i] = ch[3];
    }
    Yp[q] = make_float4(yv[0], yv[1], yv[2], yv[3]);
    Cb[q] = make_float4(cbv[0], cbv[1], cbv[2], cbv[3]);
    Cr[q] = make_float4(crv[0], crv[1], crv[2], crv[3]);
    if (D == 4) A[q] = make_float4(av[0], av[1], av[2], av[3]);
}

template <int D, bool CONV>
__global__ __launch_bounds__(256) void k_ycc_merge4(const float4* __restrict__ Yp, const float4* __restrict__ Cb,
                                                    const float4* __restrict__ Cr, const float4* __restrict__ A,
                                                    size_t n4, unsigned* __restrict__ rgb32, unsigned* __restrict__ conv32)
{
    const size_t q = (size_t)blockIdx.x * 256 + threadIdx.x;
    if (q >= n4) return;
    const float4 y4 = Yp[q], cb4 = Cb[q], cr4 = Cr[q];
    float4 a4 = make_float4(0.f, 0.f, 0.f, 0.f);
    if (D == 4) a4 = A[q];
    const float ys[4] = {y4.x, y4.y, y4.z, y4.w}, cbs[4] = {cb4.x, cb4.y, cb4.z, cb4.w};
    const float crs[4] = {cr4.x, cr4.y, cr4.z, cr4.w}, as[4] = {a4.x, a4.y, a4.z, a4.w};
    unsigned wds[D] = {};
    unsigned cw = 0;
#pragma unroll
    for (int i = 0; i < 4; ++i) {
        const float fy = ys[i], cb = cbs[i] - 128.f, cr = crs[i] - 128.f;
        unsigned char px[4];
        px[0] = to_u8_sat(fy + 45.f * cr / 32.f);
        px[1] = to_u8_sat(fy - (11.f * cb + 23.f * cr) / 32.f);
        px[2] = to_u8_sat(fy + 113.f * cb / 64.f);
        px[3] = to_u8_sat(as[i]);
#pragma unroll
        for (int k = 0; k < D; ++k) {
            const int byte = i * D + k;
            wds[byte >> 2] |= (unsigned)px[k] << (8 * (byte & 3));
        }
        cw |= (unsigned)(unsigned char)fy << (8 * i);
    }
#pragma unroll
    for (int k = 0; k < D; ++k) rgb32[q * D + k] = wds[k];
    if (CONV) conv32[q] = cw;
}

static inline bool aligned16(const void* p) { return (reinterpret_cast<uintptr_t>(p) & 15u) == 0; }

void launch_rgb_split(const unsigned char* rgb, size_t n, int d, float* Yp, float* Cb, float* Cr, float* A,
                      hipStream_t s)
{
    size_t done = 0;
    if ((d == 3 || d == 4) && n >= 1024 && aligned16(Yp) && aligned16(Cb) && aligned16(Cr) && (d == 3 || aligned16(A)) &&
        (reinterpret_cast<uintptr_t>(rgb) & 3u) == 0) {
        const size_t n4 = n / 4;
        const dim3 grid((unsigned)((n4 + 255) / 256));
        if (d == 3)
            hipLaunchKernelGGL((k_rgb_split4<3>), grid, dim3(256), 0, s, reinterpret_cast<const unsigned*>(rgb), n4,
                               reinterpret_cast<float4*>(Yp), reinterpret_cast<float4*>(Cb), reinterpret_cast<float4*>(Cr),
                               reinterpret_cast<float4*>(A));
        else
            hipLaunchKernelGGL((k_rgb_split4<4>), grid, dim3(256), 0, s, reinterpret_cast<const unsigned*>(rgb), n4,
                               reinterpret_cast<float4*>(Yp), reinterpret_cast<float4*>(Cb), reinterpret_cast<float4*>(Cr),
                               reinterpret_cast<float4*>(A));
        done = n4 * 4;
    }
    if (done < n) {
        const size_t rem = n - done;
        hipLaunchKernelGGL(k_rgb_split, dim3((unsigned)((rem + 255) / 256)), dim3(256), 0, s, rgb + done * d, rem, d,
                           Yp + done, Cb + done, Cr + done, A ? A + done : A);
    }
}

void launch_ycc_merge(const float* Yp, const float* Cb, const float* Cr, const float* A, size_t n, int d,
                      unsigned char* rgb, unsigned char* conv_opt, hipStream_t s)
{
    size_t done = 0;
    if ((d == 3 || d == 4) && n >= 1024 && aligned16(Yp) && aligned16(Cb) && aligned16(Cr) && (d == 3 || aligned16(A)) &&
        (reinterpret_cast<uintptr_t>(rgb) & 3u) == 0 && (!conv_opt || (reinterpret_cast<uintptr_t>(conv_opt) & 3u) == 0)) {
        const size_t n4 = n / 4;
        const dim3 grid((unsigned)((n4 + 255) / 256));
        const float4 *y4 = reinterpret_cast<const float4*>(Yp), *cb4 = reinterpret_cast<const float4*>(Cb);
        const float4 *cr4 = reinterpret_cast<const float4*>(Cr), *a4 = reinterpret_cast<const float4*>(A);
        unsigned* o32 = reinterpret_cast<unsigned*>(rgb);
        unsigned* c32 = reinterpret_cast<unsigned*>(conv_opt);
        if (d == 3 && conv_opt) hipLaunchKernelGGL((k_ycc_merge4<3, true>), grid, dim3(256), 0, s, y4, cb4, cr4, a4, n4, o32, c32);
        else if (d == 3) hipLaunchKernelGGL((k_ycc_merge4<3, false>), grid, dim3(256), 0, s, y4, cb4, cr4, a4, n4, o32, c32);
        else if (conv_opt) hipLaunchKernelGGL((k_ycc_merge4<4, true>), grid, dim3(256), 0, s, y4, cb4, cr4, a4, n4, o32, c32);
        else hipLaunchKernelGGL((k_ycc_merge4<4, false>), grid, dim3(256), 0, s, y4, cb4, cr4, a4, n4, o32, c32);
        done = n4 * 4;
    }
    if (done < n) {
        const size_t rem = n - done;
        hipLaunchKernelGGL(k_ycc_merge, dim3((unsigned)((rem + 255) / 256)), dim3(256), 0, s, Yp + done, Cb + done, Cr + done,
                           A ? A + done : A, rem, d, rgb + done * d, conv_opt ? conv_opt + done : conv_opt);
    }
}

}
```

### libsrcnn_amd/csrc/srcnn_pipeline.cpp

```cpp
#include <hip/hip_runtime.h>
#include <sys/mman.h>

#include <algorithm>
#include <chrono>
#include <cstdio>
#include <cstdlib>
#include <cstring>
#include <string>
#include <thread>

#include "srcnn_host.hpp"

namespace srcnn {
namespace {

struct PhaseRecord { double v[8] = {0, 0, 0, 0, 0, 0, 0, 0}; int n = 0; };
thread_local PhaseRecord g_phases;

std::atomic<unsigned> g_stream_graph_frames{0}, g_stream_plain_frames{0};
std::atomic<int> g_stream_fell_back{0};

double process_cpu_seconds()
{
    timespec ts;
// ... 167 lines not shown
        if (threaded) launched.publish(f + 1);
        else copy_frame(f);
    }
    if (rc) launched.cancel();
    if (threaded) copier.join();
    for (int i = 0; i < nslots; ++i) {
        if (cx.slots[i].st) (void)wait_stream(cx.slots[i].st);
        if (cx.slots[i].cst) (void)wait_stream(cx.slots[i].cst);
    }
    if (!rc && copy_err) rc = fail(SRCNN_E_HIP, "a device-to-host copy of the frame stream failed");
    return rc;
}

struct AsyncLink {
    std::mutex m;
    std::condition_variable cv;
    bool done = false, valid = false;
    bool leased = false;
    hipEvent_t ev = nullptr;
    int device = 0;
    void settle(bool ok)
    {
        { std::lock_guard<std::mutex> lk(m); if (done) return; done = true; leased = true; valid = ok; }
        cv.notify_all();
    }
    void mark_leased() { { std::lock_guard<std::mutex> lk(m); leased = true; } cv.notify_all(); }
    void wait_leased() { std::unique_lock<std::mutex> lk(m); cv.wait(lk, [&] { return leased; }); }
    ~AsyncLink()
    {
        if (!ev) return;
        int cur = -1;
        (void)hipGetDevice(&cur);
        (void)hipSetDevice(device);
        (void)hipEventDestroy(ev);
        if (cur >= 0) (void)hipSetDevice(cur);
    }
};

struct ProcJob {
    const unsigned char* rgb; unsigned w, h, d, dw, dh; int filter, cfilter, mode;
    unsigned char* out; unsigned char* conv;
    bool trace;
    AsyncLink* after = nullptr;
    AsyncLink* mine = nullptr;
};

std::vector<unsigned> band_starts(unsigned R0, unsigned R1, unsigned dw, unsigned dh, bool first_share_of_many, int grid, int tile_rows)
{
    const unsigned cap = budget_band_rows(dw);
    static const double seven[] = {0.05, 0.15, 0.30, 0.27, 0.16, 0.05}, six[] = {0.10, 0.30, 0.30, 0.20, 0.07}, four[] = {0.45, 0.35, 0.15};
    const size_t share_px = (size_t)(R1 - R0) * dw;
    const bool large = share_px >= 11000000u;
    const bool tiny = share_px < 3000000u;
    static const std::vector<double> env_plan = [] {
        std::vector<double> v;
        if (const char* e = settings().bands.empty() ? nullptr : settings().bands.c_str()) {
            double sum = 0;
            for (const char* q = e; *q;) {
                char* end = nullptr;
                const double f = strtod(q, &end);
                if (end == q) break;
                if (f > 0 && sum + f < 1.0 && v.size() < 15) { v.push_back(f); sum += f; }
                q = (*end == ',') ? end + 1 : end;
                if (*end != ',') break;
            }
        }
        return v;
    }();
    const bool custom = !env_plan.empty() && !first_share_of_many;
    const double* plan = custom ? env_plan.data() : (tiny ? four : (large ? seven : six));
    const int nplan = custom ? (int)env_plan.size() : (tiny ? 3 : (large ? 6 : 5));
    std::vector<unsigned> cuts = (R1 - R0 >= 512) ? plan_cuts(R0, R1, dw, dh, plan, nplan, grid, tile_rows) : std::vector<unsigned>{R0, R1};
    std::vector<unsigned> out{R0};
    for (size_t i = 1; i < cuts.size(); ++i) {
        unsigned a = out.back();
        const unsigned b = cuts[i];
        if (b <= a) continue;
        while (b - a > cap) { a += cap; out.push_back(a); }
        out.push_back(b);
    }
    return out;
}

int process_share(Ctx& cx, const ProcJob& J, unsigned R0, unsigned R1, bool one_of_many)
{
    int rc = bind(cx);
    if (rc) return rc;
    TraceRange tr("srcnn_process_u8 ctx %d rows [%u,%u) of %ux%ux%u -> %ux%u", cx.index, R0, R1, J.w, J.h, J.d, J.dw, J.dh);
    if (J.after) J.after->wait_leased();
    LaneLease lease(cx);
    if (J.mine) J.mine->mark_leased();
    if (lease.rc) return lease.rc;
    ProcLane& L = *lease.lane;
    Workspace& ws = L.ws;
    hipStream_t s = L.st;
    std::vector<TableRef> tables;
    Call c;
    c.cx = &cx; c.s = s; c.ws = &ws; c.mode = J.mode; c.hold = &tables;
    const unsigned w = J.w, h = J.h, d = J.d, dw = J.dw, dh = J.dh;
    const size_t n = (size_t)w * h;
    const auto now = [] { return std::chrono::steady_clock::now(); };
    const auto t0 = now();

    {
        const size_t need = n * d + (size_t)(R1 - R0) * dw * (d + 1 + 4 + 8) + (size_t)C2N * dw * std::min<size_t>(R1 - R0, budget_band_rows(dw)) * 4;
        const size_t have = ws.footprint() + L.pin_in_n + L.pin_out_n;
        if (have > (256u << 20) && have > 8 * need) { (void)wait_stream(L.st); (void)wait_stream(L.copy_st); L.release_buffers(); }
    }

    unsigned lo = 0, hi = h;
    TableRef cv, ch_, yv, yh;
    const bool identity = (dw == w && dh == h);
    if (!identity) {
        if ((rc = y_path_source_rows(c, h, dh, J.filter, R0, R1, lo, hi))) return rc;
        if (dh != h) {
            if ((rc = get_table(c, J.cfilter, dh, h, cv))) return rc;
            unsigned clo, chi;
            cv->source_span(R0, R1, clo, chi);
            lo = std::min(lo, clo); hi = std::max(hi, std::min(chi, h));
        } else { lo = std::min(lo, R0); hi = std::max(hi, R1); }
    }
    bool fused_shell = !settings().shell_unfused && !settings().resample_2pass && !identity && dw > w && dh > h;
    if (fused_shell) {
        if ((rc = get_table(c, J.cfilter, dw, w, ch_))) return rc;
        if ((rc = get_table(c, J.filter, dh, h, yv))) return rc;
        if ((rc = get_table(c, J.filter, dw, w, yh))) return rc;
        const unsigned ya = R0 >= 6 ? R0 - 6 : 0, yb = std::min(dh, R1 + 6);
        fused_shell = rs2d_fits(1, (int)w, (int)h, (int)dw, (int)dh, (int)ya, (int)yb, yv->view(), yh->view()) &&
                      rs2d_fits((int)d - 1, (int)w, (int)h, (int)dw, (int)dh, (int)R0, (int)R1, cv->view(), ch_->view());
    }

    const size_t share_px = (size_t)(R1 - R0) * dw;
    if ((rc = grow_ws(ws, ws.bytes, ws.bytes_n, n * d + share_px * d + share_px))) return rc;
    unsigned char* d_rgb = ws.bytes;
    unsigned char* d_out = ws.bytes + n * d;
    unsigned char* d_conv = d_out + share_px * d;
    const size_t planes_need = share_px + (fused_shell ? 0 : 4 * n + 3 * share_px);
    if ((rc = grow_ws(ws, ws.planes, ws.planes_n, planes_need))) return rc;
    float* yp = ws.planes;
    float* sp[4] = {nullptr, nullptr, nullptr, nullptr};
    float* dp[4] = {yp, nullptr, nullptr, nullptr};
    if (!fused_shell) {
        for (int k = 0; k < 4; ++k) sp[k] = ws.planes + share_px + k * n;
        for (int k = 1; k < 4; ++k) dp[k] = ws.planes + share_px + 4 * n + (k - 1) * share_px;
    }

    int grid = 0, tile_rows = 0;
    if ((J.mode & 0xff) != SRCNN_MODE_FAST_F16) conv12_grid_info(cx.num_cus, &grid, &tile_rows);
    const std::vector<unsigned> cuts = band_starts(R0, R1, dw, dh, one_of_many, grid, tile_rows);
    const unsigned nb = (unsigned)cuts.size() - 1;
    unsigned max_band = 0;
    for (unsigned b = 0; b < nb; ++b) max_band = std::max(max_band, cuts[b + 1] - cuts[b]);
    const bool no_planes = c.mode == SRCNN_MODE_FAST_F16;
    if (!no_planes && (rc = grow_ws(ws, ws.c2, ws.c2_n, (size_t)C2N * dw * std::min(dh, max_band + 4)))) return rc;
    if ((rc = grow_ws(ws, ws.up, ws.up_n, (size_t)dw * std::min(dh, max_band + 12)))) return rc;
    if (!fused_shell && (rc = grow_ws(ws, ws.tmp, ws.tmp_n, (size_t)std::max(w, dw) * std::max(h, std::min(dh, max_band + 12))))) return rc;
    while (L.band_events.size() < 3 * nb + 1) {
        hipEvent_t e;
        HIP_TRY(hipEventCreateWithFlags(&e, kBlockingEvent));
        L.band_events.push_back(e);
    }

    const size_t out_bytes = share_px * d;
    const bool small = out_bytes < (8u << 20) && !one_of_many;
    const bool in_pinned = !small && pinned_by_library(J.rgb, n * d);
    const bool out_pinned = !small && pinned_by_library(J.out, (size_t)dw * dh * d) && (!J.conv || pinned_by_library(J.conv, (size_t)dw * dh));
    const bool small_in_locked = small && pinned_by_library(J.rgb, n * d);
    const bool small_out_locked = small && pinned_by_library(J.out, (size_t)dw * dh * d) && (!J.conv || pinned_by_library(J.conv, (size_t)dw * dh));
    const size_t src_off = (size_t)lo * w * d, src_bytes = (size_t)(hi - lo) * w * d;
    unsigned staged = lo;
    unsigned n_staged = 0;
    auto stage_rows = [&](unsigned upto) -> int {
        upto = std::min(std::max(upto, staged), hi);
        if (upto == staged) return SRCNN_OK;
        const size_t off = (size_t)staged * w * d, nbytes = (size_t)(upto - staged) * w * d;
        if (small) {
            const unsigned char* from = J.rgb + off;
            if (!small_in_locked) {
                memcpy(L.pin_in + (off - src_off), J.rgb + off, nbytes);
                from = L.pin_in + (off - src_off);
            }
            HIP_TRY(hipMemcpyAsync(d_rgb + off, from, nbytes, hipMemcpyHostToDevice, s));
        } else {
            const unsigned char* from = J.rgb + off;
            if (!in_pinned) {
                parallel_memcpy(L.pin_in + (off - src_off), J.rgb + off, nbytes);
                from = L.pin_in + (off - src_off);
            }
            hipEvent_t ev = L.band_events[2 * nb + n_staged++];
            HIP_TRY(hipMemcpyAsync(d_rgb + off, from, nbytes, hipMemcpyHostToDevice, L.in_st));
            HIP_TRY(hipEventRecord(ev, L.in_st));
            if (settings().device_wait_in) HIP_TRY(hipStreamWaitEvent(s, ev, 0));
            else if (wait_event(ev) != hipSuccess) return fail(SRCNN_E_HIP, "stage-in copy");
        }
        if (!fused_shell)
            launch_rgb_split(d_rgb + off, (size_t)(upto - staged) * w, (int)d, sp[0] + (size_t)staged * w, sp[1] + (size_t)staged * w,
                             sp[2] + (size_t)staged * w, sp[3] + (size_t)staged * w, s);
        staged = upto;
        return SRCNN_OK;
    };
    auto band_source_end = [&](unsigned a, unsigned b, unsigned& upto) -> int {
        upto = hi;
        if (identity) return SRCNN_OK;
        unsigned l2 = 0, h2 = hi;
        int r = y_path_source_rows(c, h, dh, J.filter, a, b, l2, h2);
        if (r) return r;
        if (cv) { unsigned cl, chh; cv->source_span(a, b, cl, chh); h2 = std::max(h2, std::min(chh, h)); }
        else h2 = std::max(h2, std::min(b, h));
        upto = std::min(h2, hi);
        return SRCNN_OK;
    };
    std::thread prefault;
    bool prefaulting = false;
    if (small) {
        if (!small_in_locked && (rc = grow_pinned(cx, L.pin_in, L.pin_in_n, src_bytes))) return rc;
        if (!small_out_locked && (rc = grow_pinned(cx, L.pin_out, L.pin_out_n, out_bytes + share_px))) return rc;
    }
    if (!small) {
        if (!in_pinned && (rc = grow_pinned(cx, L.pin_in, L.pin_in_n, src_bytes))) return rc;
        if (!out_pinned && (rc = grow_pinned(cx, L.pin_out, L.pin_out_n, out_bytes + share_px))) return rc;
        unsigned char* o0 = J.out + (size_t)R0 * dw * d;
        unsigned char* c0 = J.conv ? J.conv + (size_t)R0 * dw : nullptr;
        if (!out_pinned) {
            hint_huge_pages(o0, out_bytes);
            if (c0) hint_huge_pages(c0, share_px);
        }
        const int pf_threads = (int)settings().prefault_threads;
        if (settings().prefault && !out_pinned) prefaulting = try_thread(prefault, [=] { prefault_pages(o0, out_bytes, pf_threads); if (c0) prefault_pages(c0, share_px); });
    }
    struct JoinPrefault {
        std::thread& t; bool& on;
        ~JoinPrefault() { if (on) t.join(); }
    } join_prefault{prefault, prefaulting};
    const auto t1 = now();

    bool chained_in = false;
    auto chain_in = [&]() -> int {
        if (chained_in || !J.after) return SRCNN_OK;
        chained_in = true;
        AsyncLink& a = *J.after;
        {
            std::unique_lock<std::mutex> lk(a.m);
            a.cv.wait(lk, [&] { return a.done; });
        }
        if (a.valid && a.ev) {
            if (settings().async_chain == 2) HIP_TRY(hipStreamWaitEvent(s, a.ev, 0));
            else if (wait_event(a.ev) != hipSuccess) return fail(SRCNN_E_HIP, "waiting for the previous asynchronous job's kernels");
        }
        return SRCNN_OK;
    };
    auto chain_out = [&]() {
        if (!J.mine) return;
        AsyncLink& m = *J.mine;
        m.device = cx.device;
        bool ok = m.ev || hipEventCreateWithFlags(&m.ev, hipEventDisableTiming) == hipSuccess;
        ok = ok && hipEventRecord(m.ev, s) == hipSuccess;
        m.settle(ok);
    };

    const YSource ysrc = fused_shell ? YSource::from_rgb(d_rgb, (int)d) : YSource::from_plane(sp[0]);
    auto run_band = [&](unsigned a, unsigned b) -> int {
        const size_t p0 = (size_t)(a - R0) * dw, pn = (size_t)(b - a) * dw;
        int r = y_path_rows(c, ysrc, w, h, dw, dh, J.filter, a, b, yp + p0);
        if (r) return r;
        if (fused_shell) {
            const DevAxisTable tv = cv->view(), th = ch_->view();
            if (!launch_merge_fused(d_rgb, (int)w, (int)h, (int)d, yp + p0, d_out + p0 * d, J.conv ? d_conv + p0 : nullptr,
                                    (int)dw, (int)dh, (int)a, (int)(b - a), tv, th, s))
                return fail(SRCNN_E_UNSUPPORTED, "fused colour shell refused a shape it was selected for");
        } else {
            for (unsigned k = 1; k < d; ++k)
                if ((r = resample_rows_range(c, sp[k], w, h, dw, dh, J.cfilter, a, b, dp[k] + p0))) return r;
            launch_ycc_merge(yp + p0, dp[1] + p0, dp[2] + p0, dp[3] ? dp[3] + p0 : nullptr, pn, (int)d, d_out + p0 * d,
                             J.conv ? d_conv + p0 : nullptr, s);
        }
        HIP_TRY(hipGetLastError());
        return SRCNN_OK;
    };

    if (small) {
        if ((rc = chain_in())) return rc;
        if ((rc = stage_rows(hi))) return rc;
        if ((rc = run_band(R0, R1))) return rc;
        chain_out();
        unsigned char* to_rgb = small_out_locked ? J.out + (size_t)R0 * dw * d : L.pin_out;
        unsigned char* to_conv = small_out_locked ? (J.conv ? J.conv + (size_t)R0 * dw : nullptr) : L.pin_out + out_bytes;
        HIP_TRY(hipMemcpyAsync(to_rgb, d_out, out_bytes, hipMemcpyDeviceToHost, s));
        if (J.conv) HIP_TRY(hipMemcpyAsync(to_conv, d_conv, share_px, hipMemcpyDeviceToHost, s));
        HIP_TRY(wait_stream(s));
        if (!small_out_locked) {
            memcpy(J.out + (size_t)R0 * dw * d, L.pin_out, out_bytes);
            if (J.conv) memcpy(J.conv + (size_t)R0 * dw, L.pin_out + out_bytes, share_px);
        }
        return SRCNN_OK;
    }

    unsigned char* pin_rgb = out_pinned ? nullptr : L.pin_out;
    unsigned char* pin_conv = out_pinned ? nullptr : L.pin_out + out_bytes;
    std::atomic<int> copy_err{0};
    std::atomic<long> us_first_queued{0}, us_kernels_done{0}, us_landed{0};
    const auto since = [&] { return (long)std::chrono::duration_cast<std::chrono::microseconds>(now() - t0).count(); };
    Handoff enqueued;
    auto d2h_band = [&](unsigned b) {
        const size_t p0 = (size_t)(cuts[b] - R0) * dw, pn = (size_t)(cuts[b + 1] - cuts[b]) * dw;
        const hipError_t kd = wait_event(L.band_events[2 * b]);
        if (b + 1 == nb) us_kernels_done = since();
        const size_t g0 = (size_t)cuts[b] * dw;
// ... 406 lines not shown
```

### libsrcnn_amd/csrc/srcnn_settings.hpp

```cpp
#pragma once
#include <cstddef>
#include <string>

#define SRCNN_SETTINGS(X)                                                                                                          \
                                                                                                            \
    X(S, devices,          "SRCNN_DEVICES",          "",    "unset = device 0, `all`, `0,1,...`", "contexts of a process that never calls `srcnn_init*` (an id may repeat: virtual contexts on one device)") \
    X(I, max_workspace_mb, "SRCNN_MAX_WORKSPACE_MB", 4608, "MiB (API twin `srcnn_set_workspace_limit`)", "layer-2 scratch one pass may hold; larger ranges are banded, bit-identically.  The default holds a whole 7680x4320 output frame (4.25 GB); lower it where memory is short: 2048 costs -1...+2 % by box, 512 +2 %, 256 +9 % (`profiles/r06_lowmem.txt`); 16384 until round 6") \
    X(I, max_lanes,        "SRCNN_MAX_LANES",        4,     "1...64", "concurrent `ProcessSRCNN` calls per context before callers queue") \
    X(B, numa,             "SRCNN_NUMA",             1,     "0/1", "place page-locked staging on the device's NUMA node (the caller's memory policy is saved and restored)") \
    X(I, comm_timeout_ms,  "SRCNN_COMM_TIMEOUT_MS",  60000, "ms, 0 = none (API twin `srcnn_comm_set_timeout_ms`)", "deadline of every wait on a peer") \
    X(B, comm_check,       "SRCNN_COMM_CHECK",       1,     "0/1", "all-reduce a checksum of every new gather table across the ranks before the first gather that uses it") \
    X(S, rccl_lib,         "SRCNN_RCCL_LIB",         "",    "path", "load this RCCL instead of the one next to the bound `libamdhip64` (site builds; the test-suite's one-device stand-in).  A trust boundary: the named file's code runs in the process; refused under secure execution (`AT_SECURE`)") \
    X(I, async_chain,      "SRCNN_ASYNC_CHAIN",      1,     "0/1/2", "order the kernels of consecutive asynchronous `ProcessSRCNN` jobs: 0 = not at all, 1 = on the host, 2 = with device-side event waits") \
    X(B, trace,            "SRCNN_TRACE",            0,     "0/1", "one stderr line per `srcnn_process_u8` share (setup / bands / stamps)") \
    X(B, roctx,            "SRCNN_ROCTX",            0,     "0/1", "roctx ranges for `rocprofv3 --marker-trace`") \
    X(S, bands,            "SRCNN_BANDS",            "",    "`f0,f1,...`", "band fractions of a large `ProcessSRCNN` image instead of the planned cuts") \
    X(I, graph_max_cpu_pct, "SRCNN_GRAPH_MAX_CPU_PCT", 10,  "0...100, 0 = never fall back", "`srcnn_y_upscale2x_f32_stream(use_graph = 1)`: hipGraph replay is kept only while the process's CPU time per replayed frame stays below this share of the frame's wall time (plain launches cost 6-8 % of a 4K frame; replay on ROCm 7.2 costs 20 % in a fresh process and ~100 % -- a runtime thread spinning from launch to completion -- in a process with more streams); above it the stream goes on with plain launches: same kernels, same overlap") \
    X(B, prefault,         "SRCNN_PREFAULT",         1,     "0/1", "pre-fault the fresh result pages of `ProcessSRCNN` in the background") \
    X(I, prefault_threads, "SRCNN_PREFAULT_THREADS", 1,     ">= 1", "helpers of that pre-faulting") \
    X(B, thp,              "SRCNN_THP",              1,     "0/1", "huge-page hint on large result blocks") \
    X(B, spin_wait,        "SRCNN_SPIN_WAIT",        0,     "0/1", "host waits through the runtime (holds a core) instead of polling") \
    X(B, device_wait_in,   "SRCNN_DEVICE_WAIT_IN",   0,     "0/1", "bands wait for their stage-in device-side (a runtime thread stays busy)") \
                   \
    X(B, conv12_queue,     "SRCNN_CONV12_QUEUE",     1,     "0/1", "layer 1+2: tiles drawn from a global counter vs dealt with a static stride") \
    X(B, conv12_dma,       "SRCNN_CONV12_DMA",       1,     "0/1", "layer 1+2: weights and Y tiles staged by LDS-DMA one tile ahead vs load, wait, `ds_write`") \
    X(B, conv12_spread,    "SRCNN_CONV12_SPREAD",    1,     "0/1", "layer 1+2: small launches dealt in quarter tiles over up to 4x more workgroups") \
    X(B, conv3_wdma,       "SRCNN_CONV3_WDMA",       1,     "0/1", "layer 3: packed weight image staged by LDS-DMA vs a plain loop") \
    X(B, conv3_off64,      "SRCNN_CONV3_OFF64",      0,     "0/1", "layer 3: 64-bit plane offsets (chosen automatically for planes of 4 GiB or more)") \
    X(B, rs_dma,           "SRCNN_RS_DMA",           1,     "0/1", "resampler: `k_rs2d_dma` (source patch by LDS-DMA) vs `k_rs2d` for plane sources") \
    X(I, rs_tpb,           "SRCNN_RS_TPB",           0,     "0 = auto, 1...16", "resampler: row tiles a block marches through") \
    X(B, resample_2pass,   "SRCNN_RESAMPLE_2PASS",   0,     "0/1", "resampler: always the two generic passes (`k_resample_cols/rows`, what down-scales use); implies the unfused colour shell") \
    X(B, shell_unfused,    "SRCNN_SHELL_UNFUSED",    0,     "0/1", "colour shell as split + plane resamples + merge instead of fused into the resampler")

namespace srcnn {

struct Settings {
#define SRCNN_SET_B(m, d) bool m = (d) != 0;
#define SRCNN_SET_I(m, d) long m = (d);
#define SRCNN_SET_S(m, d) std::string m = d;
#define X(kind, member, env, def, values, effect) SRCNN_SET_##kind(member, def)
    SRCNN_SETTINGS(X)
#undef X
#undef SRCNN_SET_B
#undef SRCNN_SET_I
#undef SRCNN_SET_S
    static Settings from_env();
    std::string describe(bool markdown) const;
};

const Settings& settings();

}
```

Baseline: 3585.

## Skip all-zero post-ReLU layer-2 channels in layer 3 via liveness bitmap

Layer 1+2 now uses wave ballots to build a per-row, per-32-column bitmap of which of the 32 ReLU outputs are nonzero, and stores it after the C2 planes in the workspace. The strict LDS-DMA layer-3 kernel ORs the bitmap over its tile window and then stages and convolves only the live channels, drawing them in groups instead of iterating all 32. This is meant to cut C2 memory traffic and FMA work in layer 3 wherever ReLU zeroes whole channels. In exchange it adds ballot and bitmap-store work in conv12, bitmap reads in conv3, and a larger workspace. Skipping exact +0.0 contributions leaves results unchanged.

Result: no change. 3569 (-0.4%).

```diff
diff --git a/include/srcnn_amd_debug.h b/include/srcnn_amd_debug.h
--- a/include/srcnn_amd_debug.h
+++ b/include/srcnn_amd_debug.h
@@ -33,6 +33,9 @@
 
 int srcnn_debug_stream_mode(unsigned* graph_frames, unsigned* plain_frames, int* fell_back);
 
+int srcnn_debug_conv12_live(const float* d_y, unsigned w, unsigned h, float* d_c2, unsigned* d_live, void* stream);
+int srcnn_debug_conv3_live(const float* d_c2, const unsigned* d_live, unsigned w, unsigned h, float* d_out, void* stream);
+
 #pragma GCC visibility pop
 #ifdef __cplusplus
 }
diff --git a/libsrcnn_amd/__init__.py b/libsrcnn_amd/__init__.py
--- a/libsrcnn_amd/__init__.py
+++ b/libsrcnn_amd/__init__.py
@@ -32,6 +32,7 @@
 DEBUG_SYMBOLS = [
     "srcnn_set_relaxation", "srcnn_axis_table", "srcnn_fused_diag", "srcnn_debug_counts", "srcnn_debug_settings",
     "srcnn_debug_clock_probe", "srcnn_debug_clock_read", "srcnn_debug_band_plan", "srcnn_debug_process_phases", "srcnn_debug_stream_mode",
+    "srcnn_debug_conv12_live", "srcnn_debug_conv3_live",
 ]
 YUV_SYMBOLS = ["srcnn_yuv_abi_version", "srcnn_yuv420_upscale_dev"]
 YUV_EX_SYMBOLS = ["srcnn_yuv_ex_abi_version", "srcnn_yuv_plane_size", "srcnn_yuv_upscale_dev"]
@@ -117,6 +118,7 @@
             "srcnn_debug_settings": (i, [C.c_char_p, sz, i]),
             "srcnn_debug_process_phases": (i, [C.POINTER(C.c_double), i]),
             "srcnn_debug_stream_mode": (i, [C.POINTER(u), C.POINTER(u), C.POINTER(i)]),
+            "srcnn_debug_conv12_live": (i, [vp, u, u, vp, vp, vp]), "srcnn_debug_conv3_live": (i, [vp, vp, u, u, vp, vp]),
             "srcnn_comm_barrier": (i, [vp]), "srcnn_comm_wait": (i, [vp]), "srcnn_comm_set_timeout_ms": (i, [i]),
             "srcnn_yuv_abi_version": (i, []),
             "srcnn_yuv420_upscale_dev": (i, [i, u, u, f, i, C.POINTER(vp), C.POINTER(sz), C.POINTER(vp), C.POINTER(sz), vp]),
@@ -406,6 +408,48 @@
     y = _plane(y)
     h, w = y.shape
     return _stage(lib().srcnn_conv12_f32_dev, y, (32, h, w), w, h)
+
+
+def live_words(w):
+    return (int(w) + 31) // 32
+
+
+def conv12_live(y):
+    y = _plane(y)
+    h, w = y.shape
+    din = DeviceBuffer.from_numpy(y)
+    dc2 = DeviceBuffer(32 * h * w * 4)
+    dlive = DeviceBuffer.from_numpy(np.full((h, live_words(w)), 0xDEADBEEF, np.uint32))
+    check(lib().srcnn_debug_conv12_live(din.ptr, w, h, dc2.ptr, dlive.ptr, None))
+    sync()
+    return dc2.to_numpy(np.float32, (32, h, w)), dlive.to_numpy(np.uint32, (h, live_words(w)))
+
+
+def conv3_live(c2, live):
+    c2 = np.ascontiguousarray(c2, np.float32)
+    _, h, w = c2.shape
+    din = DeviceBuffer.from_numpy(c2)
+    dlive = None
+    if live is not None:
+        live = np.ascontiguousarray(live, np.uint32)
+        assert live.shape == (h, live_words(w)), live.shape
+        dlive = DeviceBuffer.from_numpy(live)
+    dout = DeviceBuffer(h * w * 4)
+    check(lib().srcnn_debug_conv3_live(din.ptr, dlive.ptr if dlive else None, w, h, dout.ptr, None))
+    sync()
+    return dout.to_numpy(np.float32, (h, w))
+
+
+def live_bitmap(c2):
+    c2 = np.ascontiguousarray(c2, np.float32)
+    n, h, w = c2.shape
+    nz = c2.view(np.uint32) != 0
+    pad = live_words(w) * 32 - w
+    nz = np.pad(nz, ((0, 0), (0, 0), (0, pad))).reshape(n, h, live_words(w), 32).any(axis=3)
+    out = np.zeros((h, live_words(w)), np.uint32)
+    for m in range(n):
+        out |= nz[m].astype(np.uint32) << np.uint32(m)
+    return out
 
 
 def axis_table(dst_len, src_len, filt=SRCNNF_Bicubic):
diff --git a/libsrcnn_amd/csrc/srcnn_capi.cpp b/libsrcnn_amd/csrc/srcnn_capi.cpp
--- a/libsrcnn_amd/csrc/srcnn_capi.cpp
+++ b/libsrcnn_amd/csrc/srcnn_capi.cpp
@@ -769,7 +769,7 @@
 }
 
 void run_conv12(const Call& c, const float* Y, int W, int H, int y_row_base, int y_rows, float* C2, size_t plane, int row0,
-                int rows)
+                int rows, unsigned* live = nullptr)
 {
     unsigned long long* clk = nullptr;
     if (G.clock_probe.load(std::memory_order_relaxed) && c.cx->clock_buf)
@@ -790,7 +790,7 @@
         }
         queue = c.ws->queue;
     }
-    launch_conv12_mfma(Y, W, H, y_row_base, y_rows, C2, plane, row0, rows, c.relax(), c.cx->num_cus, c.s, clk, queue);
+    launch_conv12_mfma(Y, W, H, y_row_base, y_rows, C2, plane, row0, rows, c.relax(), c.cx->num_cus, c.s, clk, queue, live);
 }
 
 DevAxisTable view_of(const TableRef& t) { return t->view(); }
@@ -895,21 +895,22 @@
         return SRCNN_OK;
     }
 #endif
-    if ((rc = grow_ws(ws, ws.c2, ws.c2_n, (size_t)C2N * dw * (cb - ca)))) return rc;
+    if ((rc = grow_ws(ws, ws.c2, ws.c2_n, c2_elems(dw, cb - ca)))) return rc;
     TraceRange tr("srcnn y_path rows [%u,%u) of %ux%u", r0, r1, dw, dh);
     {
         StageTimer t(SRCNN_STAGE_RESAMPLE, c);
         if ((rc = resample_src_rows(c, src, w, h, dw, dh, filter, ua, ub, ws.up))) return rc;
     }
     const size_t plane = (size_t)dw * (cb - ca);
+    unsigned* live = c.relax() == 0 ? reinterpret_cast<unsigned*>(ws.c2 + (size_t)C2N * plane) : nullptr;
     {
         StageTimer t(SRCNN_STAGE_CONV12, c);
-        run_conv12(c, ws.up, (int)dw, (int)dh, (int)ua, (int)(ub - ua), ws.c2, plane, (int)ca, (int)(cb - ca));
+        run_conv12(c, ws.up, (int)dw, (int)dh, (int)ua, (int)(ub - ua), ws.c2, plane, (int)ca, (int)(cb - ca), live);
     }
     {
         StageTimer t(SRCNN_STAGE_CONV3, c);
         launch_conv3(ws.c2, plane, (int)dw, (int)dh, (int)ca, (int)(cb - ca), d_out, (int)r0, (int)(r1 - r0),
-                     c.relax(), c.s);
+                     c.relax(), c.s, live);
     }
     if (const hipError_t e = hipGetLastError(); e != hipSuccess) {
         ws.queue_dirty = true;
@@ -1846,6 +1847,32 @@
     return SRCNN_OK;
 }
 
+int srcnn_debug_conv12_live(const float* d_y, unsigned w, unsigned h, float* d_c2, unsigned* d_live, void* stream)
+{
+    int rc;
+    if ((rc = check_plane(d_y, w, h, d_c2))) return rc;
+    if (!d_live) return fail(SRCNN_E_ARG, "NULL bitmap");
+    if (h > 65535u * 4u) return fail(SRCNN_E_UNSUPPORTED, "too many rows");
+    Call c;
+    c.cx = ctx_for_stream(stream);
+    if (!c.cx) return SRCNN_E_NODEVICE;
+    c.s = (hipStream_t)stream;
+    run_conv12(c, d_y, (int)w, (int)h, 0, (int)h, d_c2, (size_t)w * h, 0, (int)h, d_live);
+    HIP_TRY(hipGetLastError());
+    return SRCNN_OK;
+}
+
+int srcnn_debug_conv3_live(const float* d_c2, const unsigned* d_live, unsigned w, unsigned h, float* d_out, void* stream)
+{
+    int rc;
+    if ((rc = check_plane(d_c2, w, h, d_out))) return rc;
+    if (h > 65535u * 16u) return fail(SRCNN_E_UNSUPPORTED, "too many rows");
+    if (!ctx_for_stream(stream)) return SRCNN_E_NODEVICE;
+    launch_conv3(d_c2, (size_t)w * h, (int)w, (int)h, 0, (int)h, d_out, 0, (int)h, 0, (hipStream_t)stream, d_live);
+    HIP_TRY(hipGetLastError());
+    return SRCNN_OK;
+}
+
 int srcnn_axis_table(int filter, unsigned dst_len, unsigned src_len, int* left, int* right, double* weights)
 {
     if (dst_len == 0 || src_len == 0) return fail(SRCNN_E_ARG, "zero length");
diff --git a/libsrcnn_amd/csrc/srcnn_kernels.h b/libsrcnn_amd/csrc/srcnn_kernels.h
--- a/libsrcnn_amd/csrc/srcnn_kernels.h
+++ b/libsrcnn_amd/csrc/srcnn_kernels.h
@@ -80,11 +80,13 @@
 hipError_t conv12_mfma_prepare();
 void launch_conv12_mfma(const float* Y, int W, int H, int y_row_base, int y_rows, float* C2, size_t plane_stride, int out_row0,
                         int out_rows, int relax, int num_cus, hipStream_t s, unsigned long long* clk = nullptr,
-                        unsigned* queue = nullptr);
+                        unsigned* queue = nullptr, unsigned* live = nullptr);
+constexpr size_t live_words(size_t W) { return (W + 31) / 32; }
+constexpr size_t c2_elems(size_t W, size_t rows) { return rows * ((size_t)C2N * W + live_words(W)); }
 void conv12_grid_info(int num_cus, int* blocks, int* tile_rows);
 constexpr int kConv12TileRows = 16, kConv12BlocksPerCU = 2;
 void launch_conv3(const float* C2, size_t plane_stride, int W, int H, int c2_row_base, int c2_rows, float* out,
-                  int out_row0, int out_rows, int relax, hipStream_t s);
+                  int out_row0, int out_rows, int relax, hipStream_t s, const unsigned* live = nullptr);
 void launch_conv1_planes(const float* Y, int W, int H, float* C1, hipStream_t s);
 void launch_conv2_planes(const float* C1, size_t n, float* C2v, hipStream_t s);
 void launch_rgb_split(const unsigned char* rgb, size_t n, int d, float* Yp, float* Cb, float* Cr, float* A,
diff --git a/libsrcnn_amd/csrc/srcnn_kernels.hip b/libsrcnn_amd/csrc/srcnn_kernels.hip
--- a/libsrcnn_amd/csrc/srcnn_kernels.hip
+++ b/libsrcnn_amd/csrc/srcnn_kernels.hip
@@ -492,7 +492,7 @@
 __global__ __launch_bounds__(64 * M_NW, 4) void k_conv12_mfma(
     const float* __restrict__ Y, int W, int H, int y_row_base, int y_rows,
     float* __restrict__ C2, size_t plane_stride, int out_row0, int out_rows, int tiles_x, int ntiles,
-    unsigned long long* __restrict__ clk, unsigned* __restrict__ queue)
+    unsigned long long* __restrict__ clk, unsigned* __restrict__ queue, unsigned* __restrict__ live, int live_stride)
 {
     constexpr int NW = M_NW, NT = 64 * NW, TH = M_TH, YT = M_YT;
     unsigned long long clk_c0 = 0, clk_r0 = 0;
@@ -675,13 +675,27 @@
             }
 
             const int row = ty0 + trow, x = tx0 + seg * 32 + col;
-            if (row < out_row0 + out_rows && row < H && x < W) {
+            const bool row_in = row < out_row0 + out_rows && row < H;
+            const bool stored = row_in && x < W;
+#pragma unroll
+            for (int r = 0; r < 16; ++r) acc2[r] = fmaxf(acc2[r] + B2s[half * 16 + r], 0.f);
+            if (stored) {
                 float* dst = C2 + (size_t)(row - out_row0) * W + x;
 #pragma unroll
                 for (int r = 0; r < 16; ++r) {
                     const int m = 8 * (r >> 2) + (r & 3);
-                    dst[(size_t)(m + 4 * half) * plane_stride] = fmaxf(acc2[r] + B2s[half * 16 + r], 0.f);
-                }
+                    dst[(size_t)(m + 4 * half) * plane_stride] = acc2[r];
+                }
+            }
+            if (live != nullptr && row_in && tx0 + seg * 32 < W) {
+                unsigned mask = 0u;
+#pragma unroll
+                for (int r = 0; r < 16; ++r) {
+                    const int m = 8 * (r >> 2) + (r & 3);
+                    const unsigned long long nz = __builtin_amdgcn_ballot_w64(stored && __float_as_uint(acc2[r]) != 0u);
+                    mask |= ((unsigned)nz != 0u ? 1u << m : 0u) | ((unsigned)(nz >> 32) != 0u ? 1u << (m + 4) : 0u);
+                }
+                if (lane == 0) live[(size_t)(row - out_row0) * (size_t)live_stride + (size_t)((tx0 >> 5) + seg)] = mask;
             }
         }
         if (dyn && tid == 0) qslot[(it + 1) & 1] = drawn;
@@ -708,7 +722,8 @@
 template <bool STRICT, bool OFF64 = false, bool X64 = false, bool SDMA = false>
 __global__ __launch_bounds__(256, SDMA ? 6 : 3) void k_conv3(
     const float* __restrict__ C2, size_t plane_stride, int W, int H, int c2_row_base, int c2_rows,
-    float* __restrict__ out, int out_row0, int out_rows, int weights_by_dma)
+    float* __restrict__ out, int out_row0, int out_rows, int weights_by_dma,
+    const unsigned* __restrict__ live, int live_stride)
 {
     constexpr int C3_MC = c3_mc(SDMA);
     constexpr int C3_BODY = C3_MC * C3_LH / 4;
@@ -763,15 +778,17 @@
     float halo4[C3_MC];
     const int h4row = min(tid >> 2, C3_LH - 1);
     const unsigned h4off = ((unsigned)row_of(h4row) * (unsigned)W + (unsigned)hx) * 4u;
-    auto issue_dma = [&](int mc, float* dst) {
+    auto chan_of = [](unsigned chs, int m) { return (int)((chs >> (8 * m)) & 0xffu); };
+    auto issue_dma = [&](unsigned chs, int n, float* dst) {
         if (tid < C3_LH * 4) {
 #pragma unroll
             for (int m = 0; m < C3_MC; ++m)
-                halo4[m] = *reinterpret_cast<const float*>(reinterpret_cast<const char*>(C2 + (size_t)(mc + m) * plane_stride) + h4off);
+                if (m < n) halo4[m] = *reinterpret_cast<const float*>(reinterpret_cast<const char*>(C2 + (size_t)chan_of(chs, m) * plane_stride) + h4off);
         }
 #pragma unroll
         for (int m = 0; m < C3_MC; ++m) {
-            const unsigned long long pb = reinterpret_cast<unsigned long long>(C2 + (size_t)(mc + m) * plane_stride);
+            if (m >= n) break;
+            const unsigned long long pb = reinterpret_cast<unsigned long long>(C2 + (size_t)chan_of(chs, m) * plane_stride);
             const unsigned ub_hi = (unsigned)__builtin_amdgcn_readfirstlane((int)(unsigned)(pb >> 32));
             const unsigned ub_lo = (unsigned)__builtin_amdgcn_readfirstlane((int)(unsigned)pb);
             const unsigned long long ub = ((unsigned long long)ub_hi << 32) | (unsigned long long)ub_lo;
@@ -783,10 +800,11 @@
             }
         }
     };
-    auto land_dma = [&](float* dst) {
+    auto land_dma = [&](int n, float* dst) {
         if (tid < C3_LH * 4) {
 #pragma unroll
-            for (int m = 0; m < C3_MC; ++m) dst[m * C3_CH + h4row * C3_LW + hlc] = halo4[m];
+            for (int m = 0; m < C3_MC; ++m)
+                if (m < n) dst[m * C3_CH + h4row * C3_LW + hlc] = halo4[m];
         }
         asm volatile("s_waitcnt vmcnt(0)" ::: "memory");
     };
@@ -816,8 +834,37 @@
 
     float sum[4] = {0.f, 0.f, 0.f, 0.f};
 
-    if constexpr (SDMA) { issue_dma(0, tile[0]); land_dma(tile[0]); }
-    else { issue(0); land(tile[0]); }
+    unsigned alive = 0xffffffffu;
+    if constexpr (STRICT && SDMA) {
+        if (live != nullptr) {
+            const int s0 = max(tx0 - 2, 0) >> 5, s1 = min(tx0 + C3_TW + 1, W - 1) >> 5;
+            unsigned a = 0u;
+#pragma unroll
+            for (int i = 0; i < (C3_LH * 4 + 63) / 64; ++i) {
+                const int e = lane + 64 * i, sg = s0 + (e & 3);
+                if (e < C3_LH * 4 && sg <= s1) a |= live[(size_t)row_of(e >> 2) * (size_t)live_stride + (size_t)sg];
+            }
+#pragma unroll
+            for (int d = 32; d >= 1; d >>= 1) a |= (unsigned)__shfl_xor((int)a, d, 64);
+            alive = (unsigned)__builtin_amdgcn_readfirstlane((int)a);
+        }
+    }
+    unsigned rem = alive;
+    auto draw = [&](int& n) {
+        unsigned chs = 0u;
+        n = 0;
+#pragma unroll
+        for (int m = 0; m < C3_MC; ++m)
+            if (rem) { chs |= (unsigned)__builtin_ctz(rem) << (8 * m); rem &= rem - 1u; ++n; }
+        return chs;
+    };
+    int cur_n, nxt_n = 0;
+    unsigned cur_chs = draw(cur_n), nxt_chs = 0u;
+
+    if (cur_n > 0) {
+        if constexpr (SDMA) { issue_dma(cur_chs, cur_n, tile[0]); land_dma(cur_n, tile[0]); }
+        else { issue(0); land(tile[0]); }
+    }
     if constexpr (STRICT) asm volatile("s_waitcnt vmcnt(0)" ::: "memory");
     __syncthreads();
 
@@ -826,17 +873,19 @@
     asm volatile("" : "+v"(offB));
 
 #pragma unroll 1
-    for (int c = 0; c < C2N / C3_MC; ++c) {
+    for (int c = 0; cur_n > 0; ++c) {
         const float* cur = tile[c & 1];
-        if (c + 1 < C2N / C3_MC) {
-            if constexpr (SDMA) issue_dma((c + 1) * C3_MC, tile[(c + 1) & 1]);
-            else issue((c + 1) * C3_MC);
+        nxt_chs = draw(nxt_n);
+        if (nxt_n > 0) {
+            if constexpr (SDMA) issue_dma(nxt_chs, nxt_n, tile[(c + 1) & 1]);
+            else issue(chan_of(nxt_chs, 0));
         }
 #pragma unroll 1
-        for (int m = 0; m < C3_MC; ++m) {
+        for (int m = 0; m < cur_n; ++m) {
+            const int ch = chan_of(cur_chs, m);
             const float* t = cur + m * C3_CH + (wv * 4) * C3_LW + lane;
             if constexpr (X64) {
-                const double* wd = reinterpret_cast<const double*>(w3s) + (c * C3_MC + m) * 25;
+                const double* wd = reinterpret_cast<const double*>(w3s) + ch * 25;
                 double a[4] = {0.0, 0.0, 0.0, 0.0};
 #pragma unroll
                 for (int r = 0; r < 8; ++r) {
@@ -872,7 +921,7 @@
                     vp[k + 4] = f2{tB[k * C3_LW + 4], tB[(k + 1) * C3_LW + 4]};
                 }
                 vp[3] = f2{tA[3 * C3_LW + 4], tB[4]};
-                const float* wrow = w3s + (c * C3_MC + m) * 30;
+                const float* wrow = w3s + ch * 30;
                 double a[4] = {0.0, 0.0, 0.0, 0.0};
 #pragma unroll
                 for (int dy = 0; dy < 5; ++dy) {
@@ -903,7 +952,7 @@
                     vb[r] = f2{t[r * C3_LW + 2], t[r * C3_LW + 3]};
                     vc[r] = t[r * C3_LW + 4];
                 }
-                const float* wrow = w3s + (c * C3_MC + m) * 30;
+                const float* wrow = w3s + ch * 30;
                 double a[4] = {0.0, 0.0, 0.0, 0.0};
 #pragma unroll
                 for (int dy = 0; dy < 5; ++dy) {
@@ -924,7 +973,7 @@
 #pragma unroll
                 for (int q = 0; q < 4; ++q) sum[q] = (float)((double)sum[q] + a[q]);
             } else {
-                const float* wm = cW.w3[c * C3_MC + m];
+                const float* wm = cW.w3[ch];
                 float win[8][5];
 #pragma unroll
                 for (int r = 0; r < 8; ++r)
@@ -941,11 +990,12 @@
                 }
             }
         }
-        if (c + 1 < C2N / C3_MC) {
-            if constexpr (SDMA) land_dma(tile[(c + 1) & 1]);
+        if (nxt_n > 0) {
+            if constexpr (SDMA) land_dma(nxt_n, tile[(c + 1) & 1]);
             else land(tile[(c + 1) & 1]);
         }
         __syncthreads();
+        cur_chs = nxt_chs; cur_n = nxt_n;
     }
     const int x = tx0 + lane;
 #pragma unroll
@@ -1296,7 +1346,7 @@
 }
 
 void launch_conv12_mfma(const float* Y, int W, int H, int y_row_base, int y_rows, float* C2, size_t plane_stride, int out_row0,
-                        int out_rows, int relax, int num_cus, hipStream_t s, unsigned long long* clk, unsigned* queue)
+                        int out_rows, int relax, int num_cus, hipStream_t s, unsigned long long* clk, unsigned* queue, unsigned* live)
 {
     if (out_rows <= 0) return;
     const int tiles_x = (int)cdiv(W, M_TW), tiles_y = (int)cdiv(out_rows, M_TH);
@@ -1304,7 +1354,7 @@
     const int cap = M_BPC * num_cus;
     const int grid = ntiles >= cap ? cap : (settings().conv12_spread ? std::min(4 * ntiles, cap) : ntiles);
 #define CONV12_GO(R, LD) hipLaunchKernelGGL((k_conv12_mfma<R, LD>), dim3(grid), dim3(64 * M_NW), sizeof(float) * m_lds_floats(LD), s, Y, W, H, \
-                                           y_row_base, y_rows, C2, plane_stride, out_row0, out_rows, tiles_x, ntiles, clk, LD ? queue : nullptr)
+                                           y_row_base, y_rows, C2, plane_stride, out_row0, out_rows, tiles_x, ntiles, clk, LD ? queue : nullptr, live, (int)cdiv(W, 32))
 #ifdef SRCNN_STRICT_ONLY
     (void)relax;
     if (settings().conv12_dma) CONV12_GO(0, true); else CONV12_GO(0, false);
@@ -1320,18 +1370,19 @@
 }
 
 void launch_conv3(const float* C2, size_t plane_stride, int W, int H, int c2_row_base, int c2_rows, float* out,
-                  int out_row0, int out_rows, int relax, hipStream_t s)
+                  int out_row0, int out_rows, int relax, hipStream_t s, const unsigned* live)
 {
     if (out_rows <= 0) return;
+    if (!settings().conv3_skip) live = nullptr;
 #ifndef SRCNN_STRICT_ONLY
     const bool strict = !(relax & (RELAX_L3_X64 | RELAX_L3_F32));
     const bool wide_planes = (size_t)c2_rows * (size_t)W * sizeof(float) >= ((size_t)1 << 32);
     if (relax & RELAX_L3_X64) {
         const dim3 gx(cdiv(W, 64), cdiv(out_rows, 16));
         if (wide_planes)
-            hipLaunchKernelGGL((k_conv3<true, true, true>), gx, dim3(256), 0, s, C2, plane_stride, W, H, c2_row_base, c2_rows, out, out_row0, out_rows, 0);
+            hipLaunchKernelGGL((k_conv3<true, true, true>), gx, dim3(256), 0, s, C2, plane_stride, W, H, c2_row_base, c2_rows, out, out_row0, out_rows, 0, nullptr, 0);
         else
-            hipLaunchKernelGGL((k_conv3<true, false, true>), gx, dim3(256), 0, s, C2, plane_stride, W, H, c2_row_base, c2_rows, out, out_row0, out_rows, 0);
+            hipLaunchKernelGGL((k_conv3<true, false, true>), gx, dim3(256), 0, s, C2, plane_stride, W, H, c2_row_base, c2_rows, out, out_row0, out_rows, 0, nullptr, 0);
         return;
     }
     if (!strict) {
@@ -1349,13 +1400,13 @@
     const bool wide = force_wide || (size_t)c2_rows * (size_t)W * sizeof(float) >= ((size_t)1 << 32);
     if (!wide && wdma)
         hipLaunchKernelGGL((k_conv3<true, false, false, true>), grid, dim3(256), 0, s, C2, plane_stride, W, H, c2_row_base, c2_rows,
-                           out, out_row0, out_rows, 1);
+                           out, out_row0, out_rows, 1, live, (int)cdiv(W, 32));
     else if (!wide)
         hipLaunchKernelGGL((k_conv3<true, false>), grid, dim3(256), 0, s, C2, plane_stride, W, H, c2_row_base, c2_rows,
-                           out, out_row0, out_rows, wdma);
+                           out, out_row0, out_rows, wdma, nullptr, 0);
     else
         hipLaunchKernelGGL((k_conv3<true, true>), grid, dim3(256), 0, s, C2, plane_stride, W, H, c2_row_base, c2_rows,
-                           out, out_row0, out_rows, wdma);
+                           out, out_row0, out_rows, wdma, nullptr, 0);
 }
 
 void launch_conv1_planes(const float* Y, int W, int H, float* C1, hipStream_t s)
diff --git a/libsrcnn_amd/csrc/srcnn_pipeline.cpp b/libsrcnn_amd/csrc/srcnn_pipeline.cpp
--- a/libsrcnn_amd/csrc/srcnn_pipeline.cpp
+++ b/libsrcnn_amd/csrc/srcnn_pipeline.cpp
@@ -343,7 +343,7 @@
     unsigned max_band = 0;
     for (unsigned b = 0; b < nb; ++b) max_band = std::max(max_band, cuts[b + 1] - cuts[b]);
     const bool no_planes = c.mode == SRCNN_MODE_FAST_F16;
-    if (!no_planes && (rc = grow_ws(ws, ws.c2, ws.c2_n, (size_t)C2N * dw * std::min(dh, max_band + 4)))) return rc;
+    if (!no_planes && (rc = grow_ws(ws, ws.c2, ws.c2_n, c2_elems(dw, std::min(dh, max_band + 4))))) return rc;
     if ((rc = grow_ws(ws, ws.up, ws.up_n, (size_t)dw * std::min(dh, max_band + 12)))) return rc;
     if (!fused_shell && (rc = grow_ws(ws, ws.tmp, ws.tmp_n, (size_t)std::max(w, dw) * std::max(h, std::min(dh, max_band + 12))))) return rc;
     while (L.band_events.size() < 3 * nb + 1) {
diff --git a/libsrcnn_amd/csrc/srcnn_settings.hpp b/libsrcnn_amd/csrc/srcnn_settings.hpp
--- a/libsrcnn_amd/csrc/srcnn_settings.hpp
+++ b/libsrcnn_amd/csrc/srcnn_settings.hpp
@@ -26,6 +26,7 @@
     X(B, conv12_dma,       "SRCNN_CONV12_DMA",       1,     "0/1", "layer 1+2: weights and Y tiles staged by LDS-DMA one tile ahead vs load, wait, `ds_write`") \
     X(B, conv12_spread,    "SRCNN_CONV12_SPREAD",    1,     "0/1", "layer 1+2: small launches dealt in quarter tiles over up to 4x more workgroups") \
     X(B, conv3_wdma,       "SRCNN_CONV3_WDMA",       1,     "0/1", "layer 3: packed weight image staged by LDS-DMA vs a plain loop") \
+    X(B, conv3_skip,       "SRCNN_CONV3_SKIP",       1,     "0/1", "layer 3: channels that are +0.0 over a tile's whole window are neither staged nor computed (liveness bitmap written by layer 1+2) vs all 32 channels for every tile") \
     X(B, conv3_off64,      "SRCNN_CONV3_OFF64",      0,     "0/1", "layer 3: 64-bit plane offsets (chosen automatically for planes of 4 GiB or more)") \
     X(B, rs_dma,           "SRCNN_RS_DMA",           1,     "0/1", "resampler: `k_rs2d_dma` (source patch by LDS-DMA) vs `k_rs2d` for plane sources") \
     X(I, rs_tpb,           "SRCNN_RS_TPB",           0,     "0 = auto, 1...16", "resampler: row tiles a block marches through") \
```
